# MVME-HBUT/Faster-OreFSDet

Measured on AMD Instinct MI355X. Metric: images/sec at 640x640 25-shot (eval FPS: model(inputs) + device sync per image, bs=1 per GPU), higher is better.
Workload: dtype f32

## Files before the change

### faster-orefsdet_amd/csrc/ore_common.h

```cpp
#pragma once
#include <hip/hip_runtime.h>
#include <stdint.h>
#include <stdio.h>
#include "ore_hip.h"

void ore_set_error(const char* fmt, ...);
void ore_note_wino(int v);
int ore_last_wino(void);
void ore_note_launch(int code, int split);
void ore_flop_count_add(double flops);

#define ORE_CHECK_ARG(cond, ...)              \
    do {                                      \
        if (!(cond)) {                        \
            ore_set_error(__VA_ARGS__);       \
            return ORE_EINVAL;                \
        }                                     \
    } while (0)

#define ORE_HIP(call)                                                                   \
    do {                                                                                \
        hipError_t e_ = (call);                                                         \
        if (e_ != hipSuccess) {                                                         \
            ore_set_error("%s:%d %s -> %s", __FILE__, __LINE__, #call, hipGetErrorString(e_)); \
            return ORE_EHIP;                                                            \
        }                                                                               \
    } while (0)

static inline int ore_launch_status(const char* what) {
    hipError_t e = hipGetLastError();
    if (e != hipSuccess) {
        ore_set_error("launch %s -> %s", what, hipGetErrorString(e));
        return ORE_EHIP;
    }
    return ORE_OK;
}

static inline int ceil_div(int a, int b) { return (a + b - 1) / b; }
static inline int round_up(int a, int b) { return ceil_div(a, b) * b; }

typedef float f32x4 __attribute__((ext_vector_type(4)));
typedef float f32x2 __attribute__((ext_vector_type(2)));
typedef __bf16 bf16x2_t __attribute__((ext_vector_type(2)));
typedef short s16x4 __attribute__((ext_vector_type(4)));
typedef unsigned u32x2 __attribute__((ext_vector_type(2)));

__device__ __forceinline__ s16x4 to_bf16x4(f32x4 v) {
    const bf16x2_t lo = __builtin_convertvector(f32x2{v.x, v.y}, bf16x2_t), hi = __builtin_convertvector(f32x2{v.z, v.w}, bf16x2_t);
    const u32x2 u = {__builtin_bit_cast(unsigned, lo), __builtin_bit_cast(unsigned, hi)};
    return __builtin_bit_cast(s16x4, u);
}

typedef __bf16 bf16x8_t __attribute__((ext_vector_type(8)));
__device__ __forceinline__ f32x4 from_bf16x4(s16x4 h) {
    const u32x2 u = __builtin_bit_cast(u32x2, h);
    return f32x4{__builtin_bit_cast(float, u.x << 16), __builtin_bit_cast(float, u.x & 0xffff0000u),
                 __builtin_bit_cast(float, u.y << 16), __builtin_bit_cast(float, u.y & 0xffff0000u)};
}
__device__ __forceinline__ float bf16_bits_to_f32(unsigned short h) { return __builtin_bit_cast(float, (unsigned)h << 16); }
struct ore_bf16_t { unsigned short v; };
__device__ __forceinline__ f32x4 ld4(const float* p) { return *reinterpret_cast<const f32x4*>(p); }
__device__ __forceinline__ f32x4 ld4(const ore_bf16_t* p) { return from_bf16x4(*reinterpret_cast<const s16x4*>(p)); }
__device__ __forceinline__ void st4(float* p, f32x4 v) { *reinterpret_cast<f32x4*>(p) = v; }
__device__ __forceinline__ void st4(ore_bf16_t* p, f32x4 v) { *reinterpret_cast<s16x4*>(p) = to_bf16x4(v); }
__device__ __forceinline__ float ld1(const float* p) { return *p; }
__device__ __forceinline__ float ld1(const ore_bf16_t* p) { return bf16_bits_to_f32(p->v); }

__device__ __forceinline__ __amdgpu_buffer_rsrc_t make_rsrc(const void* base, unsigned bytes) {
    return __builtin_amdgcn_make_buffer_rsrc(const_cast<void*>(base), 0, (int)bytes, 0x00020000);
}

__device__ __forceinline__ float ore_expf(float x) {
    if (x > 88.0f) x = 88.0f;
    if (x < -87.0f) x = -87.0f;
    const float n = rintf(x * 1.44269504088896341f);
    float r = fmaf(n, -0.693359375f, x);
    r = fmaf(n, 2.12194440e-4f, r);
    float p = 1.9875691500e-4f;
    p = fmaf(p, r, 1.3981999507e-3f);
    p = fmaf(p, r, 8.3334519073e-3f);
    p = fmaf(p, r, 4.1665795894e-2f);
    p = fmaf(p, r, 1.6666665459e-1f);
    p = fmaf(p, r, 5.0000001201e-1f);
    const float e = fmaf(p, r * r, r) + 1.0f;
    const int ni = (int)n;
    return e * __uint_as_float((unsigned)(ni + 127) << 23);
}

__device__ __forceinline__ float ore_sigmoid(float x) { return 1.0f / (1.0f + ore_expf(-x)); }

namespace oreroi {
int roi_predict_post(const float* h, int32_t C, int32_t h_parts, const float* h_bias, const float* cls_w, const float* cls_b,
                     const float* box_w, const float* box_b, const float* boxes, const int32_t* n_dev, int32_t n_host, int32_t cap,
                     const float* reg_weights4_host, float img_h, float img_w, float score_thresh, float nms_thresh,
                     int32_t topk, float* det_boxes, float* det_scores, int64_t* det_src, int32_t* det_count,
                     const float* post_dev, float* fin_boxes, float* fin_scores, int32_t* fin_count,
                     int32_t* host_count, void* workspace, size_t workspace_bytes, void* stream);
int roi_merge_classes(const float* det_boxes, const float* det_scores, const int32_t* det_count, int32_t K, int32_t cap,
                      const int64_t* class_ids, int32_t topk, const float* post_dev, float* fin_boxes, float* fin_scores,
                      int64_t* fin_classes, int32_t* fin_count, int32_t* host_count, void* stream);
struct PredictWs { size_t raw_boxes, c_boxes, raw_scores, c_scores, c_src, ok, keep, nms; };
inline PredictWs predict_ws_layout(int32_t cap) {
    const size_t c = (size_t)(cap > 0 ? cap : 1);
    PredictWs w{};
    size_t o = 256;
    w.raw_boxes = o; o += c * 16;
    w.c_boxes = o; o += c * 16;
    w.raw_scores = o; o += c * 4;
    w.c_scores = o; o += c * 4;
    w.c_src = o; o += c * 4;
    w.ok = o; o += c * 4;
    w.keep = o; o += c * 8;
    w.nms = (o + 255) & ~(size_t)255;
    return w;
}
}

namespace oremisc {
int correlation_classes(const float* q, int32_t q_ld, int32_t q_coff, int32_t n_levels, const int32_t* H, const int32_t* W, int32_t C,
                        int32_t K, const float* k11s, const float* k13s, const float* k31s, float* out, int32_t out_ld, void* stream);
int copy_cols(const float* src, int32_t src_ld, int32_t src_coff, int32_t rows, int32_t C, float* dst, int32_t dst_ld, void* stream);
}
```

### faster-orefsdet_amd/csrc/ore_detect.hip

```cpp
#include "ore_block.h"

#ifdef ORE_TRACE
__device__ unsigned long long* g_trace_det = nullptr;
#define DET_TR(i) do { if (g_trace_det && (i) < 512) g_trace_det[(i)] = __builtin_amdgcn_s_memtime(); } while (0)
__device__ int g_det_ablate = 0;
#define DET_ABL(bit) (g_det_ablate & (bit))
#else
#define DET_ABL(bit) 0
#define DET_TR(i) do { } while (0)
#endif

namespace {

struct DetP {
    int n_levels;
    const float* head[8]; int head_ld;
    int H[8], W[8], stride[8];
    float score_thresh; int pre_topk; float nms_thresh; int post_topk;
    int* lvl_cnt; float* lvl_boxes; float* lvl_scores; long long* lvl_loc;
    float* pre_boxes; float* pre_scores; long long* pre_loc; int* pre_level;
    float* s_boxes; float* s_scores; int* s_order;
    unsigned long long* mask; int mask_words;
    long long* keep_idx; int* counts; float* out_boxes; float* out_scores;
    int cap;
};

constexpr int SEL_T = 1024;
constexpr int NMS_MAX_WORDS = 256;

__device__ __forceinline__ int block_excl_scan(int v, int* lds_w, int* total) {
    const int lane = threadIdx.x & 63, wave = threadIdx.x >> 6;
    int inc = v;
#pragma unroll
    for (int d = 1; d < 64; d <<= 1) {
        const int t = __shfl_up(inc, d);
        if (lane >= d) inc += t;
    }
    __syncthreads();
    if (lane == 63) lds_w[wave] = inc;
    __syncthreads();
    int base = 0, tot = 0;
    for (int w = 0; w < SEL_T / 64; ++w) {
        const int s = lds_w[w];
        if (w < wave) base += s;
        tot += s;
    }
    *total = tot;
    return base + inc - v;
}

__device__ __forceinline__ void level_select_body(const DetP& p) {
    extern __shared__ __attribute__((aligned(16))) float sv[];
    __shared__ int hist[1024];
    __shared__ int wsum[SEL_T / 64];
    __shared__ int sh_i[4];
    const int l = blockIdx.x;
    const int HW = p.H[l] * p.W[l];
    const float* hd = p.head[l];
    const int tid = threadIdx.x;
    const bool tr = l == 0 && tid == 0;
    if (tr) DET_TR(0);

    int cnt = 0;
    for (int i = tid; i < HW; i += SEL_T) {
        const float s = ore_sigmoid(hd[(size_t)i * p.head_ld + 4]);
        sv[i] = s;
        cnt += s > p.score_thresh ? 1 : 0;
    }
    if (tr) DET_TR(1);
    int nc;
    block_excl_scan(cnt, wsum, &nc);
    if (tr) DET_TR(2);
    const int k = nc < p.pre_topk ? nc : p.pre_topk;

    unsigned T = 0;
    int quota = 0;
    bool take_all = true;
    if (nc > k) {
        take_all = false;
        unsigned prefix = 0, pmask = 0;
        int remaining = k;
        for (int pass = 0; pass < 3; ++pass) {
            const int shift = 20 - 10 * pass;
            for (int i = tid; i < 1024; i += SEL_T) hist[i] = 0;
            __syncthreads();
            for (int i = tid; i < HW; i += SEL_T) {
                const float s = sv[i];
                const unsigned key = __float_as_uint(s);
                if (s > p.score_thresh && (key & pmask) == prefix) atomicAdd(&hist[(key >> shift) & 1023], 1);
            }
            __syncthreads();
            if (tid < 64) {
                int h[16], t = 0;
#pragma unroll
                for (int j = 0; j < 16; ++j) { h[j] = hist[16 * tid + j]; t += h[j]; }
                int suf = t;
#pragma unroll
                for (int d = 1; d < 64; d <<= 1) {
                    const int o = __shfl_down(suf, d);
                    if (tid + d < 64) suf += o;
                }
                const int above = suf - t;
                if (suf >= remaining && above < remaining) {
                    int acc = above, dsel = 0, rem = remaining;
                    bool found = false;
#pragma unroll
                    for (int j = 15; j >= 0; --j) {
                        if (!found) {
                            if (acc + h[j] >= remaining) { dsel = j; rem = remaining - acc; found = true; }
                            else acc += h[j];
                        }
                    }
                    sh_i[0] = 16 * tid + dsel; sh_i[1] = rem;
                }
            }
            __syncthreads();
            prefix |= (unsigned)sh_i[0] << shift;
            pmask |= 1023u << shift;
            remaining = sh_i[1];
            if (tr) DET_TR(3 + pass);
        }
        T = prefix; quota = remaining;
    }

    const float st = (float)p.stride[l];
    const float half = (float)(p.stride[l] / 2);
    long long loc_base = 0;
    for (int j = 0; j < l; ++j) loc_base += (long long)p.H[j] * p.W[j];
    const int per = (HW + SEL_T - 1) / SEL_T;
    const int i_lo = min(tid * per, HW), i_hi = min(i_lo + per, HW);
    int my_gt = 0, my_tie = 0;
    for (int i = i_lo; i < i_hi; ++i) {
        const float s = sv[i];
        const bool cand = s > p.score_thresh;
        const unsigned key = __float_as_uint(s);
        my_gt += (cand && (take_all || key > T)) ? 1 : 0;
        my_tie += (cand && !take_all && key == T) ? 1 : 0;
    }
    if (tr) DET_TR(6);
    int tot;
    const int pre = block_excl_scan((my_gt << 16) | my_tie, wsum, &tot);
    if (tr) DET_TR(7);
    int tie_before = pre & 0xffff, gt_before = pre >> 16;
    for (int i = i_lo; i < i_hi; ++i) {
        const float s = sv[i];
        const bool cand = s > p.score_thresh;
        const unsigned key = __float_as_uint(s);
        const bool gt = cand && (take_all || key > T);
        const bool tie = cand && !take_all && key == T;
        if (gt || (tie && tie_before < quota)) {
            const int pos = gt_before + min(tie_before, quota);
            const float gx = (float)((i % p.W[l]) * p.stride[l]) + half;
            const float gy = (float)((i / p.W[l]) * p.stride[l]) + half;
            const f32x4 r = *reinterpret_cast<const f32x4*>(hd + (size_t)i * p.head_ld);
            const float x1 = gx - r.x * st, y1 = gy - r.y * st;
            float x2 = gx + r.z * st, y2 = gy + r.w * st;
            x2 = fmaxf(x2, x1 + 0.01f);
            y2 = fmaxf(y2, y1 + 0.01f);
            const size_t o = (size_t)l * p.pre_topk + pos;
            *reinterpret_cast<f32x4*>(p.lvl_boxes + o * 4) = f32x4{x1, y1, x2, y2};
            p.lvl_scores[o] = sqrtf(s);
            p.lvl_loc[o] = loc_base + i;
        }
        gt_before += gt ? 1 : 0;
        tie_before += tie ? 1 : 0;
    }
    const int out_base = (tot >> 16) + min(tot & 0xffff, quota);
    if (tid == 0) p.lvl_cnt[l] = out_base;
    if (tr) DET_TR(8);
}

__global__ __launch_bounds__(SEL_T) void k_level_select(DetP p) { level_select_body(p); }

constexpr int DET_BATCH = 16;
struct DetImg { const float* head[4]; char* ws; float* pre_boxes; float* pre_scores; long long* pre_loc; int* pre_level;
                long long* keep_idx; int* counts; float* out_boxes; float* out_scores; };
struct DetBatch {
    DetP common;
    size_t o_lvl_cnt, o_lvl_boxes, o_lvl_scores, o_lvl_loc, o_s_boxes, o_s_scores, o_s_order, o_mask;
    DetImg img[DET_BATCH];
};
__device__ __forceinline__ DetP det_of(const DetBatch& b, int i) {
    DetP p = b.common;
    const DetImg& m = b.img[i];
#pragma unroll
    for (int l = 0; l < 4; ++l) p.head[l] = m.head[l];
    p.lvl_cnt = (int*)(m.ws + b.o_lvl_cnt); p.lvl_boxes = (float*)(m.ws + b.o_lvl_boxes);
    p.lvl_scores = (float*)(m.ws + b.o_lvl_scores); p.lvl_loc = (long long*)(m.ws + b.o_lvl_loc);
    p.s_boxes = (float*)(m.ws + b.o_s_boxes); p.s_scores = (float*)(m.ws + b.o_s_scores); p.s_order = (int*)(m.ws + b.o_s_order);
    p.mask = (unsigned long long*)(m.ws + b.o_mask);
    p.pre_boxes = m.pre_boxes; p.pre_scores = m.pre_scores; p.pre_loc = m.pre_loc; p.pre_level = m.pre_level;
    p.keep_idx = m.keep_idx; p.counts = m.counts; p.out_boxes = m.out_boxes; p.out_scores = m.out_scores;
    return p;
}
__global__ __launch_bounds__(SEL_T) void k_level_select_b(DetBatch b) { const DetP p = det_of(b, blockIdx.y); level_select_body(p); }

__device__ __forceinline__ void rank_scatter_body(const DetP& p) {
    extern __shared__ float sc[];
    __shared__ int off[9];
    if (threadIdx.x == 0) {
        int a = 0;
        for (int l = 0; l < p.n_levels; ++l) { off[l] = a; a += p.lvl_cnt[l]; }
        off[p.n_levels] = a;
    }
    __syncthreads();
    const int n = off[p.n_levels];
    if (n == 0) {
        if (blockIdx.x == 0 && threadIdx.x == 0) p.counts[0] = 0;
        return;
    }
    if ((int)blockIdx.x * 16 >= n) return;
    for (int l = 0; l < p.n_levels; ++l)
        for (int i = threadIdx.x; i < off[l + 1] - off[l]; i += 256) sc[off[l] + i] = p.lvl_scores[(size_t)l * p.pre_topk + i];
    __syncthreads();
    const int e = blockIdx.x * 16 + (threadIdx.x >> 4), sub = threadIdx.x & 15;
    const bool valid = e < n;
    const float se = valid ? sc[e] : 0.f;
    int cntb = 0;
    if (valid)
        for (int f = sub; f < n; f += 16) {
            const float sf = sc[f];
            cntb += (sf > se || (sf == se && f < e)) ? 1 : 0;
        }
#pragma unroll
    for (int d = 8; d > 0; d >>= 1) cntb += __shfl_xor(cntb, d);
    if (valid && sub == 0) {
        int l = 0;
        while (e >= off[l + 1]) ++l;
        const size_t src = (size_t)l * p.pre_topk + (e - off[l]);
        const f32x4 b = *reinterpret_cast<const f32x4*>(p.lvl_boxes + src * 4);
        *reinterpret_cast<f32x4*>(p.pre_boxes + (size_t)e * 4) = b;
        p.pre_scores[e] = se;
        p.pre_loc[e] = p.lvl_loc[src];
        p.pre_level[e] = l;
        *reinterpret_cast<f32x4*>(p.s_boxes + (size_t)cntb * 4) = b;
        p.s_scores[cntb] = se;
        p.s_order[cntb] = e;
        if (e == 0) p.counts[0] = n;
    }
}

__global__ __launch_bounds__(256) void k_rank_scatter(DetP p) { rank_scatter_body(p); }
__global__ __launch_bounds__(256) void k_rank_scatter_b(DetBatch b) { const DetP p = det_of(b, blockIdx.y); rank_scatter_body(p); }

__device__ __forceinline__ void nms_mask_body(const float* __restrict__ boxes, const int* __restrict__ n_ptr,
                                              float thr, unsigned long long* __restrict__ mask, int words) {
    const int n = *n_ptr;
    const int bi = blockIdx.y, bj = blockIdx.x;
// ... 460 lines not shown

#ifdef ORE_TRACE
extern "C" int ore_debug_set_det_ablate(int flags) {
    ORE_HIP(hipMemcpyToSymbol(HIP_SYMBOL(g_det_ablate), &flags, sizeof(flags)));
    return ORE_OK;
}
extern "C" int ore_debug_set_trace_det(unsigned long long* buf) {
    ORE_HIP(hipMemcpyToSymbol(HIP_SYMBOL(g_trace_det), &buf, sizeof(buf)));
    return ORE_OK;
}
#endif

extern "C" size_t ore_detect_workspace_bytes(int32_t n_levels, int32_t pre_topk) {
    if (n_levels <= 0 || pre_topk <= 0) return 0;
    return det_layout(n_levels, pre_topk).total;
}

namespace {
static int detect_fill(const ore_detect_desc* d, DetP& p, DetLayout& lay, int& cap, size_t& sv_bytes) {
    ORE_CHECK_ARG(d && d->n_levels > 0 && d->n_levels <= 8 && d->pre_topk > 0, "ore_detect_fwd: bad args");
    ORE_CHECK_ARG(d->head_ld >= 8 && d->head_ld % 4 == 0, "ore_detect_fwd: head_ld=%d (need >= 8, %%4)", d->head_ld);
    ORE_CHECK_ARG(d->pre_boxes && d->pre_scores && d->pre_loc && d->pre_level && d->keep_idx && d->counts && d->out_boxes &&
                      d->out_scores && d->workspace, "ore_detect_fwd: null pointer");
    lay = det_layout(d->n_levels, d->pre_topk);
    if (d->workspace_bytes < lay.total) {
        ore_set_error("ore_detect_fwd: workspace %zu < %zu", d->workspace_bytes, lay.total);
        return ORE_ENOMEM;
    }
    cap = d->n_levels * d->pre_topk;
    ORE_CHECK_ARG((size_t)cap * 4 <= 150 * 1024 && lay.words <= NMS_MAX_WORDS, "ore_detect_fwd: cap %d too large", cap);
    ORE_CHECK_ARG(d->nms_thresh > 0.0f, "ore_detect_fwd: nms_thresh <= 0 (NMS disabled) is not supported");
    char* ws = (char*)d->workspace;
    p = DetP{};
    p.n_levels = d->n_levels; p.head_ld = d->head_ld;
    for (int l = 0; l < d->n_levels; ++l) {
        ORE_CHECK_ARG(d->head[l] && d->H[l] > 0 && d->W[l] > 0 && d->stride[l] > 0, "ore_detect_fwd: level %d", l);
        p.head[l] = d->head[l]; p.H[l] = d->H[l]; p.W[l] = d->W[l]; p.stride[l] = d->stride[l];
    }
    p.score_thresh = d->score_thresh; p.pre_topk = d->pre_topk; p.nms_thresh = d->nms_thresh; p.post_topk = d->post_topk;
    p.lvl_cnt = (int*)(ws + lay.lvl_cnt); p.lvl_boxes = (float*)(ws + lay.lvl_boxes);
    p.lvl_scores = (float*)(ws + lay.lvl_scores); p.lvl_loc = (long long*)(ws + lay.lvl_loc);
    p.pre_boxes = d->pre_boxes; p.pre_scores = d->pre_scores; p.pre_loc = (long long*)d->pre_loc; p.pre_level = d->pre_level;
    p.s_boxes = (float*)(ws + lay.s_boxes); p.s_scores = (float*)(ws + lay.s_scores); p.s_order = (int*)(ws + lay.s_order);
    p.mask = (unsigned long long*)(ws + lay.mask); p.mask_words = lay.words;
    p.keep_idx = (long long*)d->keep_idx; p.counts = d->counts; p.out_boxes = d->out_boxes; p.out_scores = d->out_scores;
    p.cap = cap;
    int hw_max = 0;
    for (int l = 0; l < d->n_levels; ++l) hw_max = max(hw_max, d->H[l] * d->W[l]);
    sv_bytes = (size_t)hw_max * 4;
    ORE_CHECK_ARG(sv_bytes <= 120 * 1024, "ore_detect_fwd: a level with %d locations exceeds the 30720-location LDS cache", hw_max);
    return ORE_OK;
}

static int detect_prepare(const ore_detect_desc* d, hipStream_t st, ScanArgs& sa, DetLayout& lay, int& cap) {
    DetP p{};
    size_t sv_bytes = 0;
    int rc = detect_fill(d, p, lay, cap, sv_bytes);
    if (rc) return rc;
    if (sv_bytes > 48 * 1024)
        ORE_HIP(hipFuncSetAttribute((const void*)k_level_select, hipFuncAttributeMaxDynamicSharedMemorySize, (int)sv_bytes));
    hipLaunchKernelGGL(k_level_select, dim3(d->n_levels), dim3(SEL_T), sv_bytes, st, p);
    if ((rc = ore_launch_status("k_level_select"))) return rc;
    const size_t sc_bytes = (size_t)cap * 4;
    if (sc_bytes > 64 * 1024)
        ORE_HIP(hipFuncSetAttribute((const void*)k_rank_scatter, hipFuncAttributeMaxDynamicSharedMemorySize, (int)sc_bytes));
    hipLaunchKernelGGL(k_rank_scatter, dim3(ceil_div(cap, 16)), dim3(256), sc_bytes, st, p);
    if ((rc = ore_launch_status("k_rank_scatter"))) return rc;
    if ((rc = launch_nms_mask(lay.words, cap, st, p.s_boxes, p.counts, d->nms_thresh, p.mask))) return rc;
    sa = ScanArgs{p.s_boxes, p.s_scores, p.s_order, p.counts, p.mask, p.keep_idx, p.out_boxes, p.out_scores, p.counts + 1};
    return ORE_OK;
}

static int detect_prepare_batch(const ore_detect_desc* d, int nb, hipStream_t st, ScanBatch& sb, DetLayout& lay, int& cap, bool& done) {
    done = false;
    if (nb < 2 || nb > DET_BATCH || d->n_levels > 4) return ORE_OK;
    DetBatch db{};
    size_t sv_bytes = 0;
    for (int i = 0; i < nb; ++i) {
        DetP p{};
        DetLayout li{};
        int ci = 0;
        size_t svi = 0;
        const int rc = detect_fill(d + i, p, li, ci, svi);
        if (rc) return rc;
        if (i == 0) { db.common = p; lay = li; cap = ci; sv_bytes = svi; if (nms_use_col(cap)) return ORE_OK; }
        const DetP& c = db.common;
        bool same = p.n_levels == c.n_levels && p.head_ld == c.head_ld && p.score_thresh == c.score_thresh && p.pre_topk == c.pre_topk;
        for (int l = 0; l < p.n_levels; ++l) same = same && p.H[l] == c.H[l] && p.W[l] == c.W[l] && p.stride[l] == c.stride[l];
        if (!same) return ORE_OK;
        DetImg& m = db.img[i];
        for (int l = 0; l < p.n_levels; ++l) m.head[l] = p.head[l];
        m.ws = (char*)d[i].workspace;
        m.pre_boxes = p.pre_boxes; m.pre_scores = p.pre_scores; m.pre_loc = p.pre_loc; m.pre_level = p.pre_level;
        m.keep_idx = p.keep_idx; m.counts = p.counts; m.out_boxes = p.out_boxes; m.out_scores = p.out_scores;
        sb.a[i] = ScanArgs{p.s_boxes, p.s_scores, p.s_order, p.counts, p.mask, p.keep_idx, p.out_boxes, p.out_scores, p.counts + 1};
    }
    db.o_lvl_cnt = lay.lvl_cnt; db.o_lvl_boxes = lay.lvl_boxes; db.o_lvl_scores = lay.lvl_scores; db.o_lvl_loc = lay.lvl_loc;
    db.o_s_boxes = lay.s_boxes; db.o_s_scores = lay.s_scores; db.o_s_order = lay.s_order; db.o_mask = lay.mask;
    int rc;
    if (sv_bytes > 48 * 1024)
        ORE_HIP(hipFuncSetAttribute((const void*)k_level_select_b, hipFuncAttributeMaxDynamicSharedMemorySize, (int)sv_bytes));
    hipLaunchKernelGGL(k_level_select_b, dim3(db.common.n_levels, nb), dim3(SEL_T), sv_bytes, st, db);
    if ((rc = ore_launch_status("k_level_select_b"))) return rc;
    const size_t sc_bytes = (size_t)cap * 4;
    if (sc_bytes > 64 * 1024)
        ORE_HIP(hipFuncSetAttribute((const void*)k_rank_scatter_b, hipFuncAttributeMaxDynamicSharedMemorySize, (int)sc_bytes));
    hipLaunchKernelGGL(k_rank_scatter_b, dim3(ceil_div(cap, 16), nb), dim3(256), sc_bytes, st, db);
    if ((rc = ore_launch_status("k_rank_scatter_b"))) return rc;
    hipLaunchKernelGGL(k_nms_mask_b, dim3(lay.words, lay.words, nb), dim3(256), 0, st, db, d->nms_thresh, lay.words);
    if ((rc = ore_launch_status("k_nms_mask_b"))) return rc;
    done = true;
    return ORE_OK;
}

}

extern "C" int ore_detect_fwd(const ore_detect_desc* d, void* stream) {
    ScanArgs sa{};
    DetLayout lay{};
    int cap = 0;
    hipStream_t st = (hipStream_t)stream;
    const int rc = detect_prepare(d, st, sa, lay, cap);
    if (rc) return rc;
    return launch_nms_scan(lay.words, st, sa.s_boxes, sa.s_scores, sa.s_order, sa.n_ptr, sa.mask, d->nms_thresh, d->post_topk, sa.keep_idx,
                           sa.out_boxes, sa.out_scores, sa.n_keep_out, nms_use_col(cap) ? nms_col_ld(cap) : 0);
}

extern "C" int ore_detect_batch_fwd(const ore_detect_desc* d, int32_t n_images, void* stream) {
    ORE_CHECK_ARG(d && n_images > 0, "ore_detect_batch_fwd: bad args");
    hipStream_t st = (hipStream_t)stream;
    for (int i0 = 0; i0 < n_images; i0 += SCAN_BATCH) {
        const int nb = min(SCAN_BATCH, n_images - i0);
        ScanBatch sb{};
        DetLayout lay{};
        int cap = 0;
        for (int i = 0; i < nb; ++i) {
            const ore_detect_desc* di = d + i0 + i;
            ORE_CHECK_ARG(di->n_levels == d->n_levels && di->pre_topk == d->pre_topk && di->nms_thresh == d->nms_thresh &&
                              di->post_topk == d->post_topk, "ore_detect_batch_fwd: image %d differs in levels / thresholds", i0 + i);
        }
        bool batched = false;
        { const int rc = detect_prepare_batch(d + i0, nb, st, sb, lay, cap, batched); if (rc) return rc; }
        for (int i = 0; i < nb && !batched; ++i) {
            const int rc = detect_prepare(d + i0 + i, st, sb.a[i], lay, cap);
            if (rc) return rc;
        }
        if (nms_use_col(cap) || nb == 1) {
            for (int i = 0; i < nb; ++i) {
                const ScanArgs& a = sb.a[i];
                const int rc = launch_nms_scan(lay.words, st, a.s_boxes, a.s_scores, a.s_order, a.n_ptr, a.mask, d->nms_thresh, d->post_topk,
                                               a.keep_idx, a.out_boxes, a.out_scores, a.n_keep_out, nms_use_col(cap) ? nms_col_ld(cap) : 0);
                if (rc) return rc;
            }
            continue;
        }
        sb.words = lay.words; sb.thr = d->nms_thresh; sb.post_topk = d->post_topk;
        const size_t dl = (size_t)lay.words * 64 * 8;
        const void* f = lay.words <= 64 ? (const void*)k_nms_scan_multi<1> : (lay.words <= 128 ? (const void*)k_nms_scan_multi<2> : (const void*)k_nms_scan_multi<4>);
        if (dl > 48 * 1024) ORE_HIP(hipFuncSetAttribute(f, hipFuncAttributeMaxDynamicSharedMemorySize, (int)dl));
        if (lay.words <= 64) hipLaunchKernelGGL(k_nms_scan_multi<1>, dim3(nb), dim3(256), dl, st, sb);
        else if (lay.words <= 128) hipLaunchKernelGGL(k_nms_scan_multi<2>, dim3(nb), dim3(256), dl, st, sb);
        else hipLaunchKernelGGL(k_nms_scan_multi<4>, dim3(nb), dim3(256), dl, st, sb);
        const int rc = ore_launch_status("k_nms_scan_multi");
        if (rc) return rc;
    }
    return ORE_OK;
}

namespace {
__global__ __launch_bounds__(256) void k_nms_prep(const float* __restrict__ boxes, const float* __restrict__ scores, int n_host,
                                                  const int* __restrict__ n_dev, float* s_boxes, float* s_scores, int* s_order,
                                                  int* n_out) {
    extern __shared__ float sc[];
    const int n = n_dev ? min(*n_dev, n_host) : n_host;
    for (int i = threadIdx.x; i < n; i += 256) sc[i] = scores[i];
    __syncthreads();
    const int e = blockIdx.x * 16 + (threadIdx.x >> 4), sub = threadIdx.x & 15;
    const bool valid = e < n;
// ... 79 lines not shown
```

### faster-orefsdet_amd/csrc/ore_engine.hip

```cpp
#include <map>
#include <string>
#include <vector>
#include <math.h>
#include <string.h>
#include "ore_common.h"
#include "ore_conv_internal.h"
#include <algorithm>


namespace {

struct HostTensor { std::vector<float> v; std::vector<int64_t> shape; };

struct Conv {
    float* w = nullptr; float* scale = nullptr; float* shift = nullptr;
    uint16_t* wh = nullptr;
    float* wino = nullptr;
    int Cin = 0, Cout = 0, k = 1, stride = 1, pad = 0, relu_cout = 0;
};

struct DwUnit { float* w_dw = nullptr; float* w_pw = nullptr; float* scale = nullptr; float* shift = nullptr; int C = 0, stride = 1; };

struct Buf { float* p = nullptr; int ld = 0; size_t rows = 0; };

struct Geo { int B, H, W, Hp, Wp; int h[6], w[6]; };

}

struct PrecisionScope {
    int saved;
    explicit PrecisionScope(int mode) : saved(ore_conv_get_precision()) { ore_conv_set_precision(mode); }
    ~PrecisionScope() { ore_conv_set_precision(saved); }
};

struct ore_engine {
    ore_model_cfg cfg{};
    int device = 0;
    int conv_precision = ORE_CONV_FP32;
    bool finalized = false;
    std::map<std::string, HostTensor> host;
    std::vector<void*> allocs;
    float* stem1_w = nullptr; float* stem1_scale = nullptr; float* stem1_shift = nullptr;
    Conv stem2, stem3;
    struct Block { Conv layer[8]; Conv concat; float* fc_w = nullptr; float* fc_b = nullptr; int cat_ch = 0; };
    struct Stage { Conv layer[8]; Conv concat; float* fc_w = nullptr; float* fc_b = nullptr; int in_ch, conv_ch, out_ch, cat_ch;
                   DwUnit dw[8]; Conv reduction; bool has_reduction = false; std::vector<Block> more; } stage[4];
    int blocks[4] = {1, 1, 1, 1};
    Buf icat[4][2], ycat[4];
    float* gate_blk = nullptr;
    bool depthwise = false;
    DwUnit dstem2, dstem3;
    Buf red[4];
    float* dw_scratch = nullptr; size_t dw_scratch_floats = 0;
    Conv lateral[3], output[3], conv3, tower, pred;
    float* out_wino3 = nullptr; float* out_shift3 = nullptr; size_t out_wino_stride = 0;
    uint16_t* out_wh3 = nullptr; size_t out_wh_stride = 0;
    float* gn_gamma = nullptr; float* gn_beta = nullptr;
    float* k11 = nullptr, *k13 = nullptr, *k31 = nullptr;
    HostTensor support[3];
    bool support_set[3] = {false, false, false};
    void* img_in = nullptr; size_t img_bytes = 0;
    Buf s1, s2, cat[4], sout[4], lat_all;
    Buf pcat, pos, tow, head;
    bool head_pred_valu = true;
    Buf tn;
    bool sb() const { return conv_precision == ORE_CONV_BF16S; }
    float* at(float* base, size_t elems) const { return sb() ? reinterpret_cast<float*>(reinterpret_cast<uint16_t*>(base) + elems) : base + elems; }
    float* gate[4] = {};
    float* lat_scaled[3] = {};
    float* gn_mul = nullptr, *gn_add = nullptr;
    float* ws = nullptr; size_t ws_floats = 0;
    float* ese_ws = nullptr;
    float* gn_ws = nullptr;
    float* colsum = nullptr; size_t colsum_floats = 0;
    float* pre_boxes = nullptr; float* pre_scores = nullptr; int64_t* pre_loc = nullptr; int32_t* pre_level = nullptr;
    int64_t* keep_idx = nullptr; int32_t* counts = nullptr; float* out_boxes = nullptr; float* out_scores = nullptr;
    void* det_ws = nullptr; size_t det_ws_bytes = 0;
    bool roi_set = false;
    int roi_cap = ORE_DET_RECORD_ROWS, roi_fc = 0, roi_pooled = 8, roi_topk = 100;
    float roi_score_thresh = 0.f, roi_nms_thresh = 0.9f, roi_reg_w[4] = {10.f, 10.f, 5.f, 5.f};
    float* roi_W = nullptr; float* roi_b = nullptr; float* roi_cls_w = nullptr; float* roi_cls_b = nullptr;
    float* roi_box_w = nullptr; float* roi_box_b = nullptr;
    float* roi_feat = nullptr; float* roi_h = nullptr;
    float* roi_hp = nullptr; int roi_ksplit = 1;
    float* det_boxes = nullptr; float* det_scores = nullptr; int64_t* det_src = nullptr; int32_t* det_count = nullptr;
    void* roi_ws = nullptr; size_t roi_ws_bytes = 0;
    int roi_stages = 1;
    float* casc_W[ORE_MAX_CASCADE] = {}; float* casc_b[ORE_MAX_CASCADE] = {}; float* casc_cls_w[ORE_MAX_CASCADE] = {};
    float* casc_cls_b[ORE_MAX_CASCADE] = {}; float* casc_box_w[ORE_MAX_CASCADE] = {}; float* casc_box_b[ORE_MAX_CASCADE] = {};
    float casc_reg_w[ORE_MAX_CASCADE][4] = {};
    float* casc_boxes[2] = {}; float* casc_sum = nullptr; uint8_t* casc_dead = nullptr;
    float* post = nullptr; float post_host[4] = {1.f, 1.f, 0.f, 0.f};
    char* fin_pack = nullptr; int32_t* fin_count = nullptr;
    float* fin_boxes_of(size_t b) const { return (float*)(fin_pack + b * (size_t)roi_cap * 28); }
    float* fin_scores_of(size_t b) const { return fin_boxes_of(b) + (size_t)roi_cap * 4; }
    int32_t* pin_count = nullptr; int32_t* pin_count_dev = nullptr; float* pin_post = nullptr;
    int n_classes = 0, n_slots = 0;
    int64_t* class_ids = nullptr;
    float* k11s = nullptr, *k13s = nullptr, *k31s = nullptr;
    bool slot_support_set[ORE_MAX_CLASSES][3] = {};
    float* roi_W_slot[ORE_MAX_CLASSES] = {}; float* roi_b_slot[ORE_MAX_CLASSES] = {};
    float* casc_W_slot[ORE_MAX_CLASSES][ORE_MAX_CASCADE] = {}; float* casc_b_slot[ORE_MAX_CLASSES][ORE_MAX_CASCADE] = {};
    char* det_ws_slots = nullptr;
    hipStream_t cap_stream = nullptr;
    struct GraphKey { int u8, H, W, B, K; hipGraphExec_t exec; };
    std::vector<GraphKey> graphs;
    Geo last{};
    long long pass_serial = 0;
    double last_flops = 0.0;
    bool profiling = false;
    std::vector<hipEvent_t> ev_pool;
    size_t ev_used = 0;
    struct EvSpan { size_t a, b; double flops; double flops_exec; };
    double last_profile_exec_flops = 0.0;
    std::vector<EvSpan> spans;
    hipEvent_t next_event() {
        if (ev_used == ev_pool.size()) { hipEvent_t e; if (hipEventCreate(&e) != hipSuccess) return nullptr; ev_pool.push_back(e); }
        return ev_pool[ev_used++];
    }

    template <typename T> int dalloc(T** p, size_t n) {
        void* q = nullptr;
        ORE_HIP(hipMalloc(&q, (n ? n : 1) * sizeof(T)));
        allocs.push_back(q);
        *p = (T*)q;
        return ORE_OK;
    }
    int upload(float** dst, const std::vector<float>& v) {
        int rc = dalloc(dst, v.size());
        if (rc) return rc;
// ... 292 lines not shown
                                                   reinterpret_cast<const uint16_t*>(e->sout[s].p), e->sout[s].ld, 0, g.h[k], g.w[k],
                                                   reinterpret_cast<uint16_t*>(nx.p), nx.ld, 0, st)
                      : ore_ese_gate_pool_fwd(e->colsum, cs_rows, g.h[k] * g.w[k], S.out_ch, S.fc_w, S.fc_b, e->gate[s], lw, lrows,
                                              s >= 1 ? e->lat_scaled[s - 1] : nullptr, e->sout[s].p, e->sout[s].ld, 0, g.h[k], g.w[k], nx.p,
                                              nx.ld, 0, st);
            pooled_next = true;
        } else if (cs_rows > 0 && s >= 1 && e->lat_scaled[s - 1]) {
            lat_scaled_ok[s - 1] = true;
            r.rc = sb ? ore_ese_gate_scaled_weight_bf16_fwd(e->colsum, cs_rows, g.h[k] * g.w[k], S.out_ch, S.fc_w, S.fc_b, e->gate[s], e->ese_ws,
                                                            e->lateral[s - 1].w, round_up(e->lateral[s - 1].Cout, 16),
                                                            reinterpret_cast<uint16_t*>(e->lat_scaled[s - 1]), st)
                      : ore_ese_gate_scaled_weight_fwd(e->colsum, cs_rows, g.h[k] * g.w[k], S.out_ch, S.fc_w, S.fc_b, e->gate[s], e->ese_ws,
                                                       e->lateral[s - 1].w, round_up(e->lateral[s - 1].Cout, 16), e->lat_scaled[s - 1], st);
        } else if (cs_rows > 0)
            r.rc = ore_ese_gate_from_colsum_fwd(e->colsum, cs_rows, 1, g.h[k] * g.w[k], S.out_ch, S.fc_w, S.fc_b, e->gate[s], e->ese_ws, st);
        else if (sb) { ore_set_error("bf16-storage engine: the eSE pool must come fused from the concat conv (one image per pass)"); r.rc = ORE_EINVAL; }
        else
            r.rc = ore_ese_gate_fwd(e->sout[s].p, e->sout[s].ld, 0, g.B, g.h[k] * g.w[k], S.out_ch, S.fc_w, S.fc_b, e->gate[s],
                                    e->ese_ws, st);
    }
    const int F = c.fpn_ch;
    float* lat[3];
    for (int l = 0; l < 3; ++l) lat[l] = e->at(e->lat_all.p, (size_t)lvl_row0(g, l) * F);
    const bool grouped = e->out_wino3 != nullptr || e->out_wh3 != nullptr;
    for (int l = 2; l >= 0 && !r.rc; --l) {
        const int k = l + 3, s = l + 1;
        const float* add = l < 2 ? lat[l + 1] : nullptr;
        if (lat_scaled_ok[l]) {
            Conv lc = e->lateral[l];
            lc.w = e->lat_scaled[l];
            lc.wh = reinterpret_cast<uint16_t*>(e->lat_scaled[l]);
            r.conv(lc, e->sout[s].p, e->sout[s].ld, 0, g.B, g.h[k], g.w[k], lat[l], F, 0, nullptr, nullptr, 0, add, F, 0);
        } else if (sb) {
            ore_set_error("bf16-storage engine: the lateral needs the gate-scaled weights (one image per pass)"); r.rc = ORE_EINVAL;
        } else {
            r.conv(e->lateral[l], e->sout[s].p, e->sout[s].ld, 0, g.B, g.h[k], g.w[k], lat[l], F, 0,
                   e->blocks[s] > 1 ? nullptr : e->gate[s], nullptr, 0, add, F, 0);
        }
        if (!grouped)
            r.conv(e->output[l], lat[l], F, 0, g.B, g.h[k], g.w[k], e->at(e->pcat.p, (size_t)lvl_row0(g, l) * 2 * F), 2 * F, F);
    }
    if (grouped && !r.rc) {
        const int H[3] = {g.h[3], g.h[4], g.h[5]}, W[3] = {g.w[3], g.w[4], g.w[5]};
        Conv oc = e->output[0];
        oc.wino = e->out_wino3; oc.shift = e->out_shift3;
        if (sb) oc.wh = e->out_wh3;
        r.conv_levels(oc, e->lat_all.p, F, 0, g.B, H, W, e->pcat.p, 2 * F, F, F, nullptr, nullptr, 0, false, sb ? 0 : e->out_wino_stride,
                      sb ? e->out_wh_stride : 0);
    }
    *flops = r.flops;
    return r.rc;
}

int run_heads(ore_engine* e, const Geo& g, hipStream_t st, double* flops, bool correlate = true) {
    const ore_model_cfg& c = e->cfg;
    const int F = c.fpn_ch;
    Run r{e, st};
    r.prof = e->profiling;
    const int H[3] = {g.h[3], g.h[4], g.h[5]}, W[3] = {g.w[3], g.w[4], g.w[5]};
    const int HW[3] = {H[0] * W[0], H[1] * W[1], H[2] * W[2]};
    const bool sb = e->sb();
    const double rows = (double)g.B * (HW[0] + HW[1] + HW[2]);
    if (correlate) {
        for (int l = 0; l < 3; ++l)
            if (!e->support_set[l]) { ore_set_error("support prototype for level %d not set", l + 3); return ORE_EINVAL; }
        r.rc = sb ? ore_correlation_levels_bf16_fwd(reinterpret_cast<const uint16_t*>(e->pcat.p), 2 * F, F, g.B, 3, H, W, F, e->k11, e->k13, e->k31,
                                                    reinterpret_cast<uint16_t*>(e->pcat.p), 2 * F, 0, st)
                  : ore_correlation_levels_fwd(e->pcat.p, 2 * F, F, g.B, 3, H, W, F, e->k11, e->k13, e->k31, e->pcat.p, 2 * F, 0, st);
        if (r.rc) return r.rc;
        r.flops += 2.0 * 8.0 * rows * F;
    }
    r.conv_levels(e->conv3, e->pcat.p, 2 * F, 0, g.B, H, W, e->pos.p, F, 0);
    r.conv_levels(e->tower, e->pos.p, F, 0, g.B, H, W, e->tow.p, F, 0);
    if (r.rc) return r.rc;
    if (F == 128 && e->head_pred_valu) {
        r.rc = sb ? ore_head_pred_gn_bf16_fwd(reinterpret_cast<const uint16_t*>(e->tow.p), F, g.B, 3, H, W, 32, 1e-5f, e->gn_gamma, e->gn_beta,
                                              e->pred.w, e->pred.scale, e->pred.shift, 16, e->head.p, 8, e->gn_ws, st)
                  : ore_head_pred_gn_fwd(e->tow.p, F, g.B, 3, H, W, 32, 1e-5f, e->gn_gamma, e->gn_beta, e->pred.w, e->pred.scale,
                                         e->pred.shift, 16, e->head.p, 8, e->gn_ws, st);
        r.flops += 2.0 * rows * 5.0 * F * 9.0;
        *flops = r.flops;
        return r.rc;
    }
    r.rc = sb ? ore_groupnorm_affine_levels_bf16_fwd(reinterpret_cast<const uint16_t*>(e->tow.p), F, 0, g.B, 3, HW, F, 32, 1e-5f, e->gn_gamma,
                                                     e->gn_beta, e->gn_mul, e->gn_add, e->gn_ws, st)
              : ore_groupnorm_affine_levels_fwd(e->tow.p, F, 0, g.B, 3, HW, F, 32, 1e-5f, e->gn_gamma, e->gn_beta, e->gn_mul, e->gn_add,
                                                e->gn_ws, st);
    if (r.rc) return r.rc;
    if (sb) {
        if (!r.rc) r.rc = ore_groupnorm_apply_levels_bf16_fwd(reinterpret_cast<const uint16_t*>(e->tow.p), F, 0, g.B, 3, HW, F, e->gn_mul, e->gn_add, 1,
                                                              reinterpret_cast<uint16_t*>(e->tn.p), st);
        if (r.rc) return r.rc;
        r.conv_levels(e->pred, e->tn.p, F, 0, g.B, H, W, e->head.p, 8, 0, 16, nullptr, nullptr, 0, true);
        *flops = r.flops;
        return r.rc;
    }
    r.conv_levels(e->pred, e->tow.p, F, 0, g.B, H, W, e->head.p, 8, 0, 16, e->gn_mul, e->gn_add, 1);
    *flops = r.flops;
    return r.rc;
}

void detect_desc(ore_engine* e, const Geo& g, int b, ore_detect_desc& d) {
    const ore_model_cfg& c = e->cfg;
    const size_t cap = (size_t)3 * c.pre_topk;
    d.n_levels = 3; d.head_ld = 8;
    for (int l = 0; l < 3; ++l) {
        d.head[l] = e->head.p + ((size_t)lvl_row0(g, l) + (size_t)b * g.h[l + 3] * g.w[l + 3]) * 8;
        d.H[l] = g.h[l + 3]; d.W[l] = g.w[l + 3]; d.stride[l] = c.strides[l];
    }
    d.score_thresh = c.score_thresh; d.pre_topk = c.pre_topk; d.nms_thresh = c.nms_thresh; d.post_topk = c.post_topk;
    d.pre_boxes = e->pre_boxes + b * cap * 4; d.pre_scores = e->pre_scores + b * cap; d.pre_loc = e->pre_loc + b * cap;
    d.pre_level = e->pre_level + b * cap; d.keep_idx = e->keep_idx + b * cap; d.counts = e->counts + b * 4;
    d.out_boxes = e->out_boxes + b * cap * 4; d.out_scores = e->out_scores + b * cap;
    d.workspace = e->det_ws; d.workspace_bytes = e->det_ws_bytes;
}

int run_detect(ore_engine* e, const Geo& g, hipStream_t st, int b = 0) {
    ore_detect_desc d{};
    detect_desc(e, g, b, d);
    return ore_detect_fwd(&d, st);
}

int run_detect_classes(ore_engine* e, const Geo& g, hipStream_t st, int K) {
    ore_detect_desc d[ORE_MAX_CLASSES];
    for (int k = 0; k < K; ++k) {
        d[k] = ore_detect_desc{};
        detect_desc(e, g, k, d[k]);
        if (k > 0) d[k].workspace = e->det_ws_slots + (size_t)(k - 1) * e->det_ws_bytes;
    }
    return ore_detect_batch_fwd(d, K, st);
}

static int run_roi_rows(ore_engine* e, const Geo& g, hipStream_t st, double* flops, int b, float* roi_W, float* roi_b, const float* out_boxes,
                        const int32_t* counts);

int run_roi(ore_engine* e, const Geo& g, hipStream_t st, double* flops, int b = 0, bool class_slot = false) {
    const ore_model_cfg& c = e->cfg;
    const size_t cap = (size_t)3 * c.pre_topk, rcap = (size_t)e->roi_cap;
    float* out_boxes = e->out_boxes + b * cap * 4;
    int32_t* counts = e->counts + b * 4;
    const int S = e->roi_ksplit, NS = e->roi_stages;
    const float* h = S > 1 ? e->roi_hp : e->roi_h;
    *flops = 0.0;
    const float* boxes_k = out_boxes;
    for (int k = 0; k < NS - 1; ++k) {
        float* W_k = k == 0 ? (class_slot ? e->roi_W_slot[b] : e->roi_W) : (class_slot ? e->casc_W_slot[b][k] : e->casc_W[k]);
        float* b_k = k == 0 ? (class_slot ? e->roi_b_slot[b] : e->roi_b) : (class_slot ? e->casc_b_slot[b][k] : e->casc_b[k]);
        double fl = 0.0;
        int rc = run_roi_rows(e, g, st, &fl, b, W_k, b_k, boxes_k, counts);
        if (rc) return rc;
        *flops += fl;
        float* next = e->casc_boxes[k & 1];
        rc = ore_roi_cascade_refine_fwd(h, e->roi_fc, S > 1 ? S : 0, S > 1 ? b_k : nullptr, k == 0 ? e->roi_cls_w : e->casc_cls_w[k],
                                        k == 0 ? e->roi_cls_b : e->casc_cls_b[k], k == 0 ? e->roi_box_w : e->casc_box_w[k],
                                        k == 0 ? e->roi_box_b : e->casc_box_b[k], boxes_k, counts + 1, 0, e->roi_cap,
                                        k == 0 ? e->roi_reg_w : e->casc_reg_w[k], (float)g.H, (float)g.W, next, e->casc_sum, e->casc_dead,
                                        k > 0 ? 1 : 0, st);
        if (rc) return rc;
        boxes_k = next;
    }
    const int kl = NS - 1;
    float* roi_W = kl == 0 ? (class_slot ? e->roi_W_slot[b] : e->roi_W) : (class_slot ? e->casc_W_slot[b][kl] : e->casc_W[kl]);
    float* roi_b = kl == 0 ? (class_slot ? e->roi_b_slot[b] : e->roi_b) : (class_slot ? e->casc_b_slot[b][kl] : e->casc_b[kl]);
    double fl = 0.0;
    int rc = run_roi_rows(e, g, st, &fl, b, roi_W, roi_b, boxes_k, counts);
    if (rc) return rc;
    *flops += fl;
    if (kl == 0)
        return oreroi::roi_predict_post(h, e->roi_fc, S > 1 ? S : 0, S > 1 ? roi_b : nullptr, e->roi_cls_w, e->roi_cls_b,
                                        e->roi_box_w, e->roi_box_b, out_boxes, counts + 1, 0,
                                        e->roi_cap, e->roi_reg_w, (float)g.H, (float)g.W, e->roi_score_thresh, e->roi_nms_thresh, e->roi_topk,
                                        e->det_boxes + b * rcap * 4, e->det_scores + b * rcap, e->det_src + b * rcap, e->det_count + b * 4,
// ... 107 lines not shown
extern "C" int ore_engine_set_roi_cascade(ore_engine* e, int32_t n_stages, const float* const* W_host, const float* const* b_host,
                                          int32_t fc_dim, int32_t pooled, const float* const* cls_w_host, const float* const* cls_b_host,
                                          const float* const* box_w_host, const float* const* box_b_host, const float* reg_weights4_host,
                                          float score_thresh, float nms_thresh, int32_t topk) {
    ORE_CHECK_ARG(e && W_host && b_host && cls_w_host && cls_b_host && box_w_host && box_b_host && reg_weights4_host,
                  "ore_engine_set_roi_cascade: null pointer");
    ORE_CHECK_ARG(n_stages >= 1 && n_stages <= ORE_MAX_CASCADE, "ore_engine_set_roi_cascade: %d cascade stages: the engine runs 1 .. %d", n_stages,
                  ORE_MAX_CASCADE);
    for (int k = 0; k < n_stages; ++k)
        ORE_CHECK_ARG(W_host[k] && b_host[k] && cls_w_host[k] && cls_b_host[k] && box_w_host[k] && box_b_host[k],
                      "ore_engine_set_roi_cascade: stage %d of %d: null pointer", k, n_stages);
    int rc = ore_engine_set_roi_head(e, W_host[0], b_host[0], fc_dim, pooled, cls_w_host[0], cls_b_host[0], box_w_host[0], box_b_host[0],
                                     reg_weights4_host, score_thresh, nms_thresh, topk);
    if (rc || n_stages == 1) return rc;
    const size_t K = (size_t)pooled * pooled * e->cfg.fpn_ch, cap = (size_t)e->roi_cap;
    auto up = [&](float** dst, const float* src, size_t n) -> int {
        if (!*dst && (rc = e->dalloc(dst, n))) return rc;
        ORE_HIP(hipMemcpy(*dst, src, n * sizeof(float), hipMemcpyHostToDevice));
        return ORE_OK;
    };
    for (int k = 1; k < n_stages; ++k) {
        if ((rc = up(&e->casc_W[k], W_host[k], (size_t)fc_dim * K)) || (rc = up(&e->casc_b[k], b_host[k], fc_dim)) ||
            (rc = up(&e->casc_cls_w[k], cls_w_host[k], 2 * (size_t)fc_dim)) || (rc = up(&e->casc_cls_b[k], cls_b_host[k], 2)) ||
            (rc = up(&e->casc_box_w[k], box_w_host[k], 4 * (size_t)fc_dim)) || (rc = up(&e->casc_box_b[k], box_b_host[k], 4)))
            return rc;
        for (int i = 0; i < 4; ++i) e->casc_reg_w[k][i] = reg_weights4_host[4 * k + i];
    }
    if (!e->casc_sum) {
        if ((rc = e->dalloc(&e->casc_boxes[0], cap * 4)) || (rc = e->dalloc(&e->casc_boxes[1], cap * 4)) || (rc = e->dalloc(&e->casc_sum, cap)) ||
            (rc = e->dalloc(&e->casc_dead, cap)))
            return rc;
        ORE_HIP(hipMemset(e->casc_boxes[0], 0, cap * 16));
        ORE_HIP(hipMemset(e->casc_boxes[1], 0, cap * 16));
        ORE_HIP(hipMemset(e->casc_sum, 0, cap * 4));
        ORE_HIP(hipMemset(e->casc_dead, 0, cap));
    }
    e->roi_stages = n_stages;
    ORE_HIP(hipDeviceSynchronize());
    return ORE_OK;
}

extern "C" int ore_engine_create(const ore_model_cfg* cfg, int32_t device, ore_engine** out) {
    ORE_CHECK_ARG(cfg && out, "ore_engine_create: null");
    ORE_CHECK_ARG(cfg->layers_per_block >= 1 && cfg->layers_per_block <= 8, "layers_per_block");
    ORE_CHECK_ARG(cfg->fpn_ch % 16 == 0 && cfg->max_batch >= 1 && cfg->max_h >= 32 && cfg->max_w >= 32, "bad cfg");
    for (int i = 0; i < 3; ++i) ORE_CHECK_ARG(cfg->stem_ch[i] % 16 == 0, "stem channels must be multiples of 16");
    for (int i = 0; i < 4; ++i)
        ORE_CHECK_ARG(cfg->stage_conv_ch[i] % 16 == 0 && cfg->stage_out_ch[i] % 16 == 0, "stage channels must be multiples of 16");
    ORE_HIP(hipSetDevice(device));
    ore_engine* e = new ore_engine();
    e->cfg = *cfg; e->device = device;
    e->conv_precision = ore_conv_get_precision();
    { const char* hm = getenv("ORE_HEAD_MFMA"); e->head_pred_valu = !(hm && hm[0] == '1'); }
    *out = e;
    return ORE_OK;
}

extern "C" void ore_engine_destroy(ore_engine* e) {
    if (!e) return;
    hipSetDevice(e->device);
    for (auto& g : e->graphs) hipGraphExecDestroy(g.exec);
    if (e->cap_stream) hipStreamDestroy(e->cap_stream);
    for (auto ev : e->ev_pool) hipEventDestroy(ev);
    for (void* p : e->allocs) hipFree(p);
    if (e->pin_count) hipHostFree(e->pin_count);
    if (e->pin_post) hipHostFree(e->pin_post);
    delete e;
}

extern "C" int ore_engine_set_tensor(ore_engine* e, const char* name, const float* data, const int64_t* shape, int32_t ndim) {
    ORE_CHECK_ARG(e && name && data && ndim >= 0 && ndim <= 8, "ore_engine_set_tensor: bad args");
    ORE_CHECK_ARG(!e->finalized, "ore_engine_set_tensor: engine already finalized");
    HostTensor t;
    size_t n = 1;
    for (int i = 0; i < ndim; ++i) { t.shape.push_back(shape[i]); n *= (size_t)shape[i]; }
    t.v.assign(data, data + n);
    e->host[name] = std::move(t);
    return ORE_OK;
}

extern "C" int ore_engine_set_support(ore_engine* e, int32_t level, const float* proto, int32_t C, int32_t s) {
    ORE_CHECK_ARG(e && proto && level >= 3 && level <= 5 && C == e->cfg.fpn_ch && s >= 1, "ore_engine_set_support: bad args");
    const int l = level - 3;
    e->support[l].v.assign(proto, proto + (size_t)C * s * s);
    e->support[l].shape = {C, s, s};
    if (e->finalized) {
        ORE_HIP(hipSetDevice(e->device));
        float* tmp = nullptr;
        ORE_HIP(hipMalloc((void**)&tmp, (size_t)C * s * s * sizeof(float)));
        hipError_t err = hipMemcpy(tmp, proto, (size_t)C * s * s * sizeof(float), hipMemcpyHostToDevice);
        int rc = err == hipSuccess ? ore_support_kernels_fwd(tmp, C, s, e->k11 + (size_t)l * C, e->k13 + (size_t)l * C * 3,
                                                             e->k31 + (size_t)l * C * 3, nullptr) : ORE_EHIP;
        hipDeviceSynchronize();
        hipFree(tmp);
        if (rc) return rc;
    }
    e->support_set[l] = true;
    return ORE_OK;
}

extern "C" int ore_engine_set_depthwise(ore_engine* e, int32_t on) {
    ORE_CHECK_ARG(e && !e->finalized, "ore_engine_set_depthwise: call it before ore_engine_finalize");
    ORE_CHECK_ARG(!on || !e->sb(), "ore_engine_set_depthwise: a bf16-storage engine has no depthwise body (the depthwise units are fp32 only)");
    ORE_CHECK_ARG(!on || (e->blocks[0] == 1 && e->blocks[1] == 1 && e->blocks[2] == 1 && e->blocks[3] == 1),
                  "ore_engine_set_depthwise: this engine has identity blocks (ore_engine_set_blocks): there is no deep depthwise body");
    e->depthwise = on != 0;
// ... 123 lines not shown
        if ((rc = e->upload(&p.w, packed))) return rc;
        p.Cin = F; p.Cout = 5; p.k = 3; p.stride = 1; p.pad = 1; p.relu_cout = 4;
        if ((rc = make_bf16_w(e, &p, w5.data()))) return rc;
        std::vector<float> scale(3 * 16, 0.f), shift(3 * 16, 0.f);
        for (int l = 0; l < 3; ++l) {
            const HostTensor* sc;
            if ((rc = need(e, hp + "scales." + std::to_string(l) + ".scale", &sc, {1}))) return rc;
            const float s = sc->v[0];
            for (int j = 0; j < 4; ++j) { scale[l * 16 + j] = s; shift[l * 16 + j] = br->v[j] * s; }
            scale[l * 16 + 4] = 1.0f; shift[l * 16 + 4] = bh->v[0];
        }
        if ((rc = e->upload(&p.scale, scale)) || (rc = e->upload(&p.shift, shift))) return rc;
    }
    const Geo g = make_geo(c.max_batch, c.max_h, c.max_w);
    const size_t B = g.B;
    e->img_bytes = B * 3 * (size_t)c.max_h * c.max_w * sizeof(float);
    ORE_HIP(hipMalloc(&e->img_in, e->img_bytes));
    e->allocs.push_back(e->img_in);
    if ((rc = alloc_buf(e, &e->s1, B * g.h[1] * g.w[1], c.stem_ch[0]))) return rc;
    if ((rc = alloc_buf(e, &e->s2, B * g.h[1] * g.w[1], c.stem_ch[1]))) return rc;
    size_t cmax = 0, cs_need = 0;
    for (int s = 0; s < 4; ++s) {
        const int k = s + 2;
        const size_t M = B * g.h[k] * g.w[k];
        if ((rc = alloc_buf(e, &e->cat[s], M, e->stage[s].cat_ch))) return rc;
        if ((rc = alloc_buf(e, &e->sout[s], M, e->stage[s].out_ch))) return rc;
        if (e->stage[s].has_reduction && (rc = alloc_buf(e, &e->red[s], M, e->stage[s].conv_ch))) return rc;
        if (e->depthwise && ore_dwpw_prefers_composition((int64_t)M, e->stage[s].conv_ch, 1))
            e->dw_scratch_floats = std::max(e->dw_scratch_floats, M * (size_t)e->stage[s].conv_ch);
        if ((rc = e->dalloc(&e->gate[s], B * e->stage[s].out_ch))) return rc;
        if (e->blocks[s] > 1) {
            const int icw = e->stage[s].out_ch + c.layers_per_block * e->stage[s].conv_ch;
            if ((rc = alloc_buf(e, &e->ycat[s], M, e->stage[s].out_ch)) || (rc = alloc_buf(e, &e->icat[s][0], M, icw))) return rc;
            if (e->blocks[s] > 2 && (rc = alloc_buf(e, &e->icat[s][1], M, icw))) return rc;
            const std::vector<float> ones(B * e->stage[s].out_ch, 1.0f);
            ORE_HIP(hipMemcpy(e->gate[s], ones.data(), ones.size() * sizeof(float), hipMemcpyHostToDevice));
        } else if (s >= 1 && (rc = e->dalloc(&e->lat_scaled[s - 1], (size_t)round_up(e->cfg.fpn_ch, 16) * e->stage[s].out_ch))) return rc;
        if ((size_t)e->stage[s].out_ch > cmax) cmax = e->stage[s].out_ch;
        const size_t cs = (M / 16 + 1) * (size_t)e->stage[s].out_ch;
        if (cs > cs_need) cs_need = cs;
    }
    if (e->depthwise) {
        const size_t m1 = B * g.h[1] * g.w[1];
        if (ore_dwpw_prefers_composition((int64_t)m1, c.stem_ch[1], 1)) e->dw_scratch_floats = std::max(e->dw_scratch_floats, m1 * (size_t)c.stem_ch[1]);
        if (e->dw_scratch_floats && (rc = e->dalloc(&e->dw_scratch, e->dw_scratch_floats))) return rc;
    }
    size_t rows_all = 0;
    for (int l = 0; l < 3; ++l) rows_all += (size_t)B * g.h[l + 3] * g.w[l + 3];
    if ((rc = alloc_buf(e, &e->lat_all, rows_all, F))) return rc;
    if ((rc = alloc_buf(e, &e->pcat, rows_all, 2 * F)) || (rc = alloc_buf(e, &e->pos, rows_all, F)) ||
        (rc = alloc_buf(e, &e->tow, rows_all, F)) || (rc = alloc_buf(e, &e->head, rows_all, 8, false))) return rc;
    if (e->sb() && (rc = alloc_buf(e, &e->tn, rows_all, F))) return rc;
    ORE_HIP(hipMemset(e->head.p, 0, rows_all * 8 * sizeof(float)));
    if ((rc = e->dalloc(&e->gn_mul, 3 * B * F)) || (rc = e->dalloc(&e->gn_add, 3 * B * F))) return rc;
    if ((rc = e->dalloc(&e->k11, (size_t)3 * F)) || (rc = e->dalloc(&e->k13, (size_t)3 * F * 3)) || (rc = e->dalloc(&e->k31, (size_t)3 * F * 3))) return rc;
    e->ws_floats = ore_conv_workspace_floats();
    if ((rc = e->dalloc(&e->ws, e->ws_floats))) return rc;
    ORE_HIP(hipMemset(e->ws, 0, e->ws_floats * sizeof(float)));
    if ((rc = e->dalloc(&e->ese_ws, B * (ORE_ESE_PARTS + 1) * cmax))) return rc;
    if (std::any_of(e->blocks, e->blocks + 4, [](int n) { return n > 1; }) && (rc = e->dalloc(&e->gate_blk, B * cmax))) return rc;
    e->colsum_floats = cs_need;
    if ((rc = e->dalloc(&e->colsum, cs_need))) return rc;
    if ((rc = e->dalloc(&e->gn_ws, (rows_all / 64 + 3 * B + 8) * 64 * 2))) return rc;
    const size_t cap = (size_t)3 * c.pre_topk;
    const size_t MB = (size_t)c.max_batch;
    if ((rc = e->dalloc(&e->pre_boxes, MB * cap * 4)) || (rc = e->dalloc(&e->pre_scores, MB * cap)) || (rc = e->dalloc(&e->pre_loc, MB * cap)) ||
        (rc = e->dalloc(&e->pre_level, MB * cap)) || (rc = e->dalloc(&e->keep_idx, MB * cap)) || (rc = e->dalloc(&e->counts, MB * 4)) ||
        (rc = e->dalloc(&e->out_boxes, MB * cap * 4)) || (rc = e->dalloc(&e->out_scores, MB * cap))) return rc;
    ORE_HIP(hipMemset(e->counts, 0, MB * 4 * sizeof(int32_t)));
    e->det_ws_bytes = ore_detect_workspace_bytes(3, c.pre_topk);
    char* dws = nullptr;
    if ((rc = e->dalloc(&dws, e->det_ws_bytes))) return rc;
    e->det_ws = dws;
    ORE_HIP(hipStreamCreateWithFlags(&e->cap_stream, hipStreamNonBlocking));
    e->finalized = true;
    for (int l = 0; l < 3; ++l)
        if (!e->support[l].v.empty()) {
            e->support_set[l] = false;
            if ((rc = ore_engine_set_support(e, l + 3, e->support[l].v.data(), (int)e->support[l].shape[0], (int)e->support[l].shape[1]))) return rc;
        }
    e->host.clear();
    ORE_HIP(hipDeviceSynchronize());
    return ORE_OK;
}

static int check_geo(ore_engine* e, int B, int H, int W) {
    ORE_CHECK_ARG(e && e->finalized, "engine not finalized");
    ORE_CHECK_ARG(B >= 1 && B <= e->cfg.max_batch && H >= 1 && W >= 1 && round_up(H, 32) <= round_up(e->cfg.max_h, 32) &&
                      round_up(W, 32) <= round_up(e->cfg.max_w, 32) &&
                      (size_t)B * round_up(H, 32) * round_up(W, 32) <= (size_t)e->cfg.max_batch * round_up(e->cfg.max_h, 32) * round_up(e->cfg.max_w, 32),
                  "input %dx%dx%d exceeds the engine's max %dx%dx%d", B, H, W, e->cfg.max_batch, e->cfg.max_h, e->cfg.max_w);
    return ORE_OK;
}

template <typename Body>
static int replay_or_capture(ore_engine* e, int is_u8, int H, int W, int B, int K, hipStream_t st, Body& body) {
    for (auto& k : e->graphs)
        if (k.u8 == is_u8 && k.H == H && k.W == W && k.B == B && k.K == K) {
            ORE_HIP(hipGraphLaunch(k.exec, st));
            return ORE_OK;
        }
    hipGraph_t graph = nullptr;
    const bool was_prof = e->profiling;
    e->profiling = false;
    ORE_HIP(hipStreamBeginCapture(e->cap_stream, hipStreamCaptureModeThreadLocal));
    int rc = body(e->cap_stream, &e->last_flops);
// ... 51 lines not shown

extern "C" int ore_engine_detect_begin(ore_engine* e, const void* img, int32_t is_u8, int32_t H, int32_t W, int32_t out_h, int32_t out_w,
                                       void* out_record, void* stream) {
    return detect_begin(e, img, is_u8, H, W, out_h, out_w, out_record, stream, false);
}

extern "C" int ore_engine_detect_end(ore_engine* e, void* stream, int32_t* n_det) {
    ORE_CHECK_ARG(e && e->roi_set && n_det, "ore_engine_detect_end: null");
    hipStream_t st = (hipStream_t)stream;
    volatile unsigned long long* rec_word = reinterpret_cast<volatile unsigned long long*>(e->pin_count) + 1;
    volatile int32_t* cnt_word = e->pin_count;
    ORE_CHECK_ARG(*rec_word != 0ull, "ore_engine_detect_end: no ore_engine_detect_begin is pending on this engine");
    int32_t n = -1;
    for (int spin = 0; spin < (1 << 22); ++spin) {
        n = *cnt_word;
        if (n >= 0) break;
        __builtin_ia32_pause();
    }
    if (n < 0) {
        const hipError_t se = hipStreamSynchronize(st);
        if (se != hipSuccess) { *rec_word = 0ull; ore_set_error("ore_engine_detect_end: %s", hipGetErrorString(se)); return ORE_EHIP; }
        n = *cnt_word;
        if (n < 0) { *rec_word = 0ull; ore_set_error("ore_engine_detect_end: the pass finished without writing the detection count"); return ORE_EHIP; }
    }
    __atomic_thread_fence(__ATOMIC_ACQUIRE);
    *rec_word = 0ull;
    *n_det = n;
    return ORE_OK;
}

extern "C" int ore_engine_detect_fwd(ore_engine* e, const void* img, int32_t is_u8, int32_t H, int32_t W, int32_t out_h, int32_t out_w,
                                     void* out_record, void* stream, int32_t* n_det) {
    ORE_CHECK_ARG(n_det, "ore_engine_detect_fwd: null count");
    const int rc = ore_engine_detect_begin(e, img, is_u8, H, W, out_h, out_w, out_record, stream);
    return rc ? rc : ore_engine_detect_end(e, stream, n_det);
}

extern "C" int ore_engine_eval_batch_fwd(ore_engine* e, const void* img, int32_t is_u8, int32_t B, int32_t H, int32_t W,
                                         int32_t use_graph, void* stream) {
    int rc = check_geo(e, B, H, W);
    if (rc) return rc;
    ORE_CHECK_ARG(img, "null image");
    hipStream_t st = (hipStream_t)stream;
    const Geo g = make_geo(B, H, W);
    e->last = g; ++e->pass_serial;
    PrecisionScope ps(e->sb() ? ORE_CONV_FP32 : e->conv_precision);
    const size_t bytes = (size_t)B * 3 * H * W * (is_u8 ? 1 : 4);
    ORE_CHECK_ARG(bytes <= e->img_bytes, "image batch exceeds the engine's input buffer");
    if (img != e->img_in) ORE_HIP(hipMemcpyAsync(e->img_in, img, bytes, hipMemcpyDefault, st));
    auto body = [&](hipStream_t s, double* fl) -> int {
        double f1 = 0, f2 = 0;
        int r = run_backbone(e, e->img_in, is_u8, g, s, &f1);
        double f3 = 0;
        if (!r) r = run_heads(e, g, s, &f2);
        for (int b = 0; b < B && !r; ++b) {
            double fb = 0;
            r = run_detect(e, g, s, b);
            if (!r && e->roi_set) r = run_roi(e, g, s, &fb, b);
            f3 += fb;
        }
        *fl = f1 + f2 + f3;
        return r;
    };
    if (!use_graph) return body(st, &e->last_flops);
    return replay_or_capture(e, is_u8, H, W, B, 0, st, body);
}

static int eval_classes(ore_engine* e, const void* img, int32_t is_u8, int32_t H, int32_t W, int32_t use_graph, hipStream_t st) {
    ORE_CHECK_ARG(e && e->finalized, "engine not finalized");
    const int K = e->n_classes;
    ORE_CHECK_ARG(K >= 1, "N-way pass: no class set (ore_engine_set_classes with n >= 1 first)");
    for (int k = 0; k < K; ++k) {
        for (int l = 0; l < 3; ++l)
            ORE_CHECK_ARG(e->slot_support_set[k][l], "N-way pass: class slot %d has no support prototype for level %d (ore_engine_set_support_slot)", k, l + 3);
        ORE_CHECK_ARG(!e->roi_set || e->roi_W_slot[k], "N-way pass: class slot %d has no second-stage support (ore_engine_set_roi_support_slot)", k);
        for (int sk = 1; sk < e->roi_stages && e->roi_set; ++sk)
            ORE_CHECK_ARG(e->casc_W_slot[k][sk], "N-way pass: class slot %d has no second-stage support for stage %d of the %d cascade stages "
                          "(ore_engine_set_roi_support_slot_stage)", k, sk, e->roi_stages);
    }
    int rc = check_geo(e, K, H, W);
    if (rc) return rc;
    ORE_CHECK_ARG(img, "null image");
    const Geo g1 = make_geo(1, H, W), gK = make_geo(K, H, W);
    e->last = gK; ++e->pass_serial;
    PrecisionScope ps(e->conv_precision);
    const size_t bytes = (size_t)3 * H * W * (is_u8 ? 1 : 4);
    ORE_CHECK_ARG(bytes <= e->img_bytes, "image exceeds the engine's input buffer");
    if (img != e->img_in) ORE_HIP(hipMemcpyAsync(e->img_in, img, bytes, hipMemcpyDefault, st));
    const int F = e->cfg.fpn_ch;
    auto body = [&](hipStream_t s, double* fl) -> int {
        double f1 = 0, f2 = 0, f3 = 0;
        int r = run_backbone(e, e->img_in, is_u8, g1, s, &f1);
        const int rows1 = lvl_row0(g1, 3);
        const int Hl[3] = {g1.h[3], g1.h[4], g1.h[5]}, Wl[3] = {g1.w[3], g1.w[4], g1.w[5]};
        if (!r) r = oremisc::copy_cols(e->pcat.p, 2 * F, F, rows1, F, e->tow.p, F, s);
        if (!r) r = oremisc::correlation_classes(e->tow.p, F, 0, 3, Hl, Wl, F, K, e->k11s, e->k13s, e->k31s, e->pcat.p, 2 * F, s);
        f2 += 2.0 * 8.0 * (double)K * rows1 * F;
        double fh = 0;
        if (!r) r = run_heads(e, gK, s, &fh, false);
        f2 += fh;
        if (!r) r = run_detect_classes(e, gK, s, K);
        for (int k = 0; k < K && !r && e->roi_set; ++k) {
            double fb = 0;
            r = run_roi(e, gK, s, &fb, k, true);
            f3 += fb;
        }
        if (!r && e->roi_set)
// ... 134 lines not shown
extern "C" int ore_event_pair_overhead_us(void* stream, int32_t reps, double* median_us) {
    ORE_CHECK_ARG(median_us && reps >= 1 && reps <= 4096, "ore_event_pair_overhead_us: bad args");
    hipStream_t st = (hipStream_t)stream;
    std::vector<hipEvent_t> ev(2 * (size_t)reps);
    for (auto& e : ev) ORE_HIP(hipEventCreate(&e));
    double T[2] = {0.0, 0.0};
    for (int nk = 1; nk <= 2; ++nk) {
        for (int i = 0; i < 8; ++i) hipLaunchKernelGGL(k_noop, dim3(256), dim3(256), 0, st);
        for (int i = 0; i < reps; ++i) {
            ORE_HIP(hipEventRecord(ev[2 * i], st));
            for (int k = 0; k < nk; ++k) hipLaunchKernelGGL(k_noop, dim3(256), dim3(256), 0, st);
            ORE_HIP(hipEventRecord(ev[2 * i + 1], st));
        }
        ORE_HIP(hipStreamSynchronize(st));
        std::vector<float> t((size_t)reps);
        for (int i = 0; i < reps; ++i) ORE_HIP(hipEventElapsedTime(&t[i], ev[2 * i], ev[2 * i + 1]));
        std::sort(t.begin(), t.end());
        T[nk - 1] = 1e3 * (double)t[t.size() / 2];
    }
    for (auto& e : ev) (void)hipEventDestroy(e);
    const double o = 2.0 * T[0] - T[1];
    *median_us = o > 0.0 ? o : 0.0;
    return ORE_OK;
}

extern "C" int ore_engine_buffer(ore_engine* e, const char* name, void** ptr, int64_t dims[4]) {
    ORE_CHECK_ARG(e && e->finalized && name && ptr && dims, "ore_engine_buffer: bad args");
    const Geo& g = e->last;
    const std::string n(name);
    const int F = e->cfg.fpn_ch;
    auto set = [&](void* p, int64_t rows, int64_t ch, int64_t ld, int64_t coff) {
        *ptr = p; dims[0] = rows; dims[1] = ch; dims[2] = ld; dims[3] = coff; return ORE_OK;
    };
    const int64_t cap = (int64_t)3 * e->cfg.pre_topk;
    if (n == "stem1") return set(e->s1.p, (int64_t)g.B * g.h[1] * g.w[1], e->cfg.stem_ch[0], e->s1.ld, 0);
    if (n == "stem2") return set(e->s2.p, (int64_t)g.B * g.h[1] * g.w[1], e->cfg.stem_ch[1], e->s2.ld, 0);
    if (n == "stem3") return set(e->cat[0].p, (int64_t)g.B * g.h[2] * g.w[2], e->cfg.stem_ch[2], e->cat[0].ld, 0);
    for (int s = 0; s < 4; ++s) {
        const int64_t rows = (int64_t)g.B * g.h[s + 2] * g.w[s + 2];
        if (n == "stage" + std::to_string(s + 2)) return set(e->sout[s].p, rows, e->stage[s].out_ch, e->sout[s].ld, 0);
        if (n == "gate" + std::to_string(s + 2)) return set(e->gate[s], g.B, e->stage[s].out_ch, e->stage[s].out_ch, 0);
        if (n == "cat" + std::to_string(s + 2)) return set(e->cat[s].p, rows, e->stage[s].cat_ch, e->cat[s].ld, 0);
    }
    for (int l = 0; l < 3; ++l) {
        const std::string k = std::to_string(l + 3);
        const int64_t rows = (int64_t)g.B * g.h[l + 3] * g.w[l + 3];
        const size_t r0 = (size_t)lvl_row0(g, l);
        if (n == "p" + k) return set(e->at(e->pcat.p, r0 * 2 * F), rows, F, 2 * F, F);
        if (n == "attn" + k) return set(e->at(e->pcat.p, r0 * 2 * F), rows, F, 2 * F, 0);
        if (n == "lat" + k) return set(e->at(e->lat_all.p, r0 * F), rows, F, F, 0);
        if (n == "pos" + k) return set(e->at(e->pos.p, r0 * F), rows, F, F, 0);
        if (n == "tower" + k) return set(e->at(e->tow.p, r0 * F), rows, F, F, 0);
        if (n == "head" + k) return set(e->head.p + r0 * 8, rows, 5, 8, 0);
    }
    size_t ib = 0;
    std::string base = n;
    { const size_t h = n.find('#'); if (h != std::string::npos) { base = n.substr(0, h); ib = (size_t)std::atoi(n.c_str() + h + 1); } }
    if (ib >= (size_t)e->cfg.max_batch) { ore_set_error("ore_engine_buffer: image index in '%s' exceeds max_batch", name); return ORE_EINVAL; }
    const size_t ucap = (size_t)cap, rcap = (size_t)e->roi_cap;
    if (base == "pre_boxes") return set(e->pre_boxes + ib * ucap * 4, cap, 4, 4, 0);
    if (base == "pre_scores") return set(e->pre_scores + ib * ucap, cap, 1, 1, 0);
    if (base == "pre_loc") return set(e->pre_loc + ib * ucap, cap, 1, 1, 0);
    if (base == "pre_level") return set(e->pre_level + ib * ucap, cap, 1, 1, 0);
    if (base == "keep_idx") return set(e->keep_idx + ib * ucap, cap, 1, 1, 0);
    if (base == "counts") return set(e->counts + ib * 4, 4, 1, 1, 0);
    if (base == "out_boxes") return set(e->out_boxes + ib * ucap * 4, cap, 4, 4, 0);
    if (base == "out_scores") return set(e->out_scores + ib * ucap, cap, 1, 1, 0);
    if (e->roi_set) {
        if (base == "det_boxes") return set(e->det_boxes + ib * rcap * 4, e->roi_cap, 4, 4, 0);
        if (base == "det_scores") return set(e->det_scores + ib * rcap, e->roi_cap, 1, 1, 0);
        if (base == "det_src") return set(e->det_src + ib * rcap, e->roi_cap, 1, 1, 0);
        if (base == "det_count") return set(e->det_count + ib * 4, 4, 1, 1, 0);
        if (base == "final_boxes") return set(e->fin_boxes_of(ib), e->roi_cap, 4, 4, 0);
        if (base == "final_scores") return set(e->fin_scores_of(ib), e->roi_cap, 1, 1, 0);
        if (base == "final_count") return set(e->fin_count + ib * 4, 4, 1, 1, 0);
        if (base == "final_classes") return set(e->fin_pack + ib * rcap * 28 + rcap * 20, e->roi_cap, 1, 1, 0);
        if (n == "roi_h" && e->roi_ksplit <= 1) return set(e->roi_h, e->roi_cap, e->roi_fc, e->roi_fc, 0);
        const oreroi::PredictWs L = oreroi::predict_ws_layout(e->roi_cap);
        if (n == "roi_raw_boxes") return set((float*)((char*)e->roi_ws + L.raw_boxes), e->roi_cap, 4, 4, 0);
        if (n == "roi_raw_scores") return set((float*)((char*)e->roi_ws + L.raw_scores), e->roi_cap, 1, 1, 0);
        if (n == "roi_ok") return set((float*)((char*)e->roi_ws + L.ok), e->roi_cap, 1, 1, 0);
    }
    ore_set_error("ore_engine_buffer: unknown buffer '%s'", name);
    return ORE_ENOENT;
}

extern "C" int ore_engine_last_geometry(ore_engine* e, int32_t out[16]) {
    ORE_CHECK_ARG(e && e->finalized && out, "ore_engine_last_geometry: bad args");
    const Geo& g = e->last;
    out[0] = g.B; out[1] = g.H; out[2] = g.W;
    for (int l = 0; l < 3; ++l) { out[3 + 3 * l] = g.h[l + 3]; out[4 + 3 * l] = g.w[l + 3]; out[5 + 3 * l] = e->cfg.strides[l]; }
    out[12] = (int32_t)(e->pass_serial & 0x7fffffffLL); out[13] = (int32_t)(e->pass_serial >> 31);
    out[14] = out[15] = 0;
    return ORE_OK;
}

extern "C" int32_t ore_engine_buffer_is_bf16(ore_engine* e, const char* name) {
    if (!e || !name || !e->sb()) return 0;
    const std::string n(name);
    for (const char* pre : {"stem", "stage", "cat", "attn", "lat", "pos", "tower"})
        if (n.rfind(pre, 0) == 0) return 1;
    return n.size() == 2 && n[0] == 'p' ? 1 : 0;
}
```

### faster-orefsdet_amd/csrc/ore_misc.hip

```cpp
#include "ore_common.h"
#include "ore_ese.h"
#include <stdlib.h>
#include <algorithm>

namespace {

template <typename T, int NT, typename TO = float>
__global__ __launch_bounds__(256) void k_stem1(const T* __restrict__ img, int B, int H, int W, int Ho, int Wo,
                                               float m0, float m1, float m2, float s0, float s1, float s2,
                                               const float* __restrict__ w, const float* __restrict__ scale,
                                               const float* __restrict__ shift, int Cout, TO* __restrict__ out,
                                               int out_ld, int out_coff, int groups_per_wave) {
    constexpr int MAXNT = NT;
    const int lane = threadIdx.x & 63, wave = threadIdx.x >> 6;
    const int li = lane & 15, g = lane >> 4;
    int kdy[7], kdx[7], koff[7];
    bool kv[7];
    float kmean[7], kstd[7];
#pragma unroll
    for (int j = 0; j < 7; ++j) {
        const int k = 4 * j + g;
        kv[j] = k < 27;
        const int kk = kv[j] ? k : 0;
        const int kc = kk / 9;
// ... 375 lines not shown
struct GnSeg { int nlev, B; int HW[4]; int row0[4]; int chunk0[4]; int nchunk[4]; };

__device__ __forceinline__ void gn_locate_chunk(const GnSeg& g, int chunk, int& seg, int& HW, int& row0, int& local) {
    int l = 0;
#pragma unroll
    for (int j = 1; j < 4; ++j)
        if (j < g.nlev && chunk >= g.chunk0[j]) l = j;
    const int within = chunk - g.chunk0[l];
    const int b = within / g.nchunk[l];
    local = within - b * g.nchunk[l];
    HW = g.HW[l];
    row0 = g.row0[l] + b * HW;
    seg = l * g.B + b;
}

__global__ __launch_bounds__(256) void k_gn_chunk_stats(const float* __restrict__ x, int ld, int coff, GnSeg sg, int C, int G,
                                                        float* __restrict__ stats ) {
    __shared__ float red[256];
    __shared__ float gmean[64];
    int seg, HW, row0, chunk;
    gn_locate_chunk(sg, blockIdx.x, seg, HW, row0, chunk);
    const int cpg = C / G;
    const int rpar = 256 / C;
    const int c = threadIdx.x % C, rr = threadIdx.x / C;
    const int r0 = chunk * GN_ROWS, r1 = min(r0 + GN_ROWS, HW);
    const float* base = x + (size_t)row0 * ld + coff + c;
    float s = 0.f;
    for (int r = r0 + rr; r < r1; r += rpar) s += base[(size_t)r * ld];
    red[threadIdx.x] = s;
    __syncthreads();
    if (threadIdx.x < G) {
        float t = 0.f;
        for (int k = 0; k < rpar; ++k)
            for (int j = 0; j < cpg; ++j) t += red[k * C + threadIdx.x * cpg + j];
        gmean[threadIdx.x] = t / (float)((r1 - r0) * cpg);
    }
    __syncthreads();
    const float mu = gmean[c / cpg];
    float v = 0.f;
    for (int r = r0 + rr; r < r1; r += rpar) { const float d = base[(size_t)r * ld] - mu; v += d * d; }
    red[threadIdx.x] = v;
    __syncthreads();
    if (threadIdx.x < G) {
        float t = 0.f;
        for (int k = 0; k < rpar; ++k)
            for (int j = 0; j < cpg; ++j) t += red[k * C + threadIdx.x * cpg + j];
        float* o = stats + ((size_t)blockIdx.x * G + threadIdx.x) * 2;
        o[0] = gmean[threadIdx.x]; o[1] = t;
    }
}

template <int RPT, typename TS = float>
__global__ __launch_bounds__(256) void k_gn_chunk_stats4(const TS* __restrict__ x, int ld, int coff, GnSeg sg, int G,
                                                         float* __restrict__ stats ) {
    __shared__ float red[256];
    __shared__ float gmean[64];
    int seg, HW, row0, chunk;
    gn_locate_chunk(sg, blockIdx.x, seg, HW, row0, chunk);
    const int g = threadIdx.x % G, rr = threadIdx.x / G, rpar = 256 / G;
    const int r0 = chunk * GN_ROWS, r1 = min(r0 + GN_ROWS, HW);
    const TS* base = x + (size_t)row0 * ld + coff + g * 4;
    f32x4 v[RPT];
    float s = 0.f;
#pragma unroll
    for (int k = 0; k < RPT; ++k) {
        const int r = r0 + rr + k * rpar;
        v[k] = r < r1 ? ld4(base + (size_t)r * ld) : f32x4{0.f, 0.f, 0.f, 0.f};
        s += (v[k].x + v[k].y) + (v[k].z + v[k].w);
    }
    red[threadIdx.x] = s;
    __syncthreads();
    if (threadIdx.x < G) {
        float t = 0.f;
        for (int k = 0; k < rpar; ++k) t += red[k * G + threadIdx.x];
        gmean[threadIdx.x] = t / (float)((r1 - r0) * 4);
    }
    __syncthreads();
    const float mu = gmean[g];
    float q = 0.f;
#pragma unroll
    for (int k = 0; k < RPT; ++k) {
        if (r0 + rr + k * rpar < r1) {
            const float a = v[k].x - mu, b = v[k].y - mu, c = v[k].z - mu, d = v[k].w - mu;
            q += (a * a + b * b) + (c * c + d * d);
        }
    }
    red[threadIdx.x] = q;
    __syncthreads();
    if (threadIdx.x < G) {
        float t = 0.f;
        for (int k = 0; k < rpar; ++k) t += red[k * G + threadIdx.x];
        float* o = stats + ((size_t)blockIdx.x * G + threadIdx.x) * 2;
        o[0] = gmean[threadIdx.x]; o[1] = t;
    }
}

struct GnCombineSm { float sn[8][64], sm[8][64], sq[8][64], fmean[64], frstd[64]; };
__device__ __forceinline__ void gn_combine_block(GnCombineSm& S, const float* __restrict__ stats, const GnSeg& sg, int b, int C, int G, float eps,
                                                 const float* __restrict__ gamma, const float* __restrict__ beta, float* omul, float* oadd) {
    const int lvl = b / sg.B, img = b - lvl * sg.B;
    const int nchunks = sg.nchunk[lvl], HW = sg.HW[lvl];
    stats += (size_t)(sg.chunk0[lvl] + img * nchunks) * G * 2;
    const int cpg = C / G;
    const int gdiv = G > 32 ? 64 : 32, nsl = 256 / gdiv;
    const int g = threadIdx.x % gdiv, sl = threadIdx.x / gdiv;
    float n = 0.f, mean = 0.f, m2 = 0.f;
    if (g < G)
        for (int c0 = sl; c0 < nchunks; c0 += nsl * 8) {
            float2 rec[8];
// ... 6 lines not shown
            for (int k = 0; k < 8; ++k) {
                const int ch = c0 + nsl * k;
                if (ch < nchunks) {
                    const float nb = (float)((min((ch + 1) * GN_ROWS, HW) - ch * GN_ROWS) * cpg);
                    const float mb = rec[k].x, qb = rec[k].y;
                    const float nt = n + nb, d = mb - mean;
                    mean += d * (nb / nt);
                    m2 += qb + d * d * (n * nb / nt);
                    n = nt;
                }
            }
        }
    S.sn[sl][g] = n; S.sm[sl][g] = mean; S.sq[sl][g] = m2;
    __syncthreads();
    if (threadIdx.x < G) {
        float N = S.sn[0][g], M = S.sm[0][g], Q = S.sq[0][g];
        for (int k = 1; k < nsl; ++k) {
            const float nb = S.sn[k][g];
            if (nb > 0.f) {
                const float nt = N + nb, d = S.sm[k][g] - M;
                M += d * (nb / nt);
                Q += S.sq[k][g] + d * d * (N * nb / nt);
                N = nt;
            }
        }
        S.fmean[g] = M;
        S.frstd[g] = 1.0f / sqrtf(Q / N + eps);
    }
    __syncthreads();
    for (int c = threadIdx.x; c < C; c += 256) {
        const float m = S.frstd[c / cpg] * gamma[c];
        omul[c] = m;
        oadd[c] = beta[c] - S.fmean[c / cpg] * m;
    }
}

__global__ __launch_bounds__(256) void k_gn_combine(const float* __restrict__ stats, GnSeg sg, int C, int G, float eps,
                                                    const float* __restrict__ gamma, const float* __restrict__ beta,
                                                    float* __restrict__ mul, float* __restrict__ add) {
    __shared__ GnCombineSm S;
    const int b = blockIdx.x;
    gn_combine_block(S, stats, sg, b, C, G, eps, gamma, beta, mul + (size_t)b * C, add + (size_t)b * C);
}


struct HeadP {
    const void* tow; int ld;
    int B, nlev; int H[4], W[4], row0[4], tile0[5], tx[4], ty[4];
    const float* mul; const float* add;
    const float* w;
    const float* scale; const float* shift; int ep_stride;
    float* out; int out_ld;
    const float* stats; GnSeg sg; const float* gamma; const float* beta; float eps; int G;
};

template <typename TS>
__global__ __launch_bounds__(256) void k_head_pred(HeadP p) {
    constexpr int C = 128, Q = 32, NO = 5, TP = 8, HP = TP + 2;
    __shared__ __attribute__((aligned(16))) float sX[HP * HP * C];
    __shared__ __attribute__((aligned(16))) float sW[NO * 9 * C];
    const int tid = threadIdx.x;
    int lvl = 0;
#pragma unroll
    for (int l = 1; l < 4; ++l)
        if (l < p.nlev && (int)blockIdx.x >= p.tile0[l]) lvl = l;
    const int H = p.H[lvl], W = p.W[lvl];
    const int tl = blockIdx.x - p.tile0[lvl], per = p.tx[lvl] * p.ty[lvl];
    const int b = tl / per, tr = tl - b * per;
    const int y0 = (tr / p.tx[lvl]) * TP, x0 = (tr % p.tx[lvl]) * TP;
    const int base = p.row0[lvl] + b * H * W;
    const TS* tow = reinterpret_cast<const TS*>(p.tow);
    __shared__ __attribute__((aligned(16))) float s_mul[C], s_add[C];
    __shared__ GnCombineSm S;
    constexpr int NX = (HP * HP * Q + 255) / 256;
    constexpr int NWV = (NO * 9 * Q + 255) / 256;
    f32x4 xv[NX], wv[NWV];
#pragma unroll
    for (int k = 0; k < NWV; ++k) {
        const int i = tid + k * 256;
        wv[k] = i < NO * 9 * Q ? *reinterpret_cast<const f32x4*>(p.w + i * 4) : f32x4{0.f, 0.f, 0.f, 0.f};
    }
#pragma unroll
    for (int k = 0; k < NX; ++k) {
        const int i = tid + k * 256;
        const int px = i / Q, q = i - px * Q;
        const int gy = y0 - 1 + px / HP, gx = x0 - 1 + px % HP;
        const bool ok = i < HP * HP * Q && (unsigned)gy < (unsigned)H && (unsigned)gx < (unsigned)W;
        xv[k] = ok ? ld4(tow + (size_t)(base + gy * W + gx) * p.ld + q * 4) : f32x4{0.f, 0.f, 0.f, 0.f};
    }
    if (p.stats) gn_combine_block(S, p.stats, p.sg, lvl * p.B + b, C, p.G, p.eps, p.gamma, p.beta, s_mul, s_add);
    else if (tid < C) { s_mul[tid] = p.mul[(size_t)(lvl * p.B + b) * C + tid]; s_add[tid] = p.add[(size_t)(lvl * p.B + b) * C + tid]; }
    __syncthreads();
    const float* mul = s_mul;
    const float* add = s_add;
#pragma unroll
    for (int k = 0; k < NWV; ++k) {
        const int i = tid + k * 256;
        if (i < NO * 9 * Q) *reinterpret_cast<f32x4*>(sW + i * 4) = wv[k];
    }
#pragma unroll
    for (int k = 0; k < NX; ++k) {
        const int i = tid + k * 256;
        if (i < HP * HP * Q) {
            const int px = i / Q, q = i - px * Q;
            const int gy = y0 - 1 + px / HP, gx = x0 - 1 + px % HP;
            f32x4 v = {0.f, 0.f, 0.f, 0.f};
            if ((unsigned)gy < (unsigned)H && (unsigned)gx < (unsigned)W) {
                v = xv[k] * *reinterpret_cast<const f32x4*>(mul + q * 4) + *reinterpret_cast<const f32x4*>(add + q * 4);
                v.x = fmaxf(v.x, 0.f); v.y = fmaxf(v.y, 0.f); v.z = fmaxf(v.z, 0.f); v.w = fmaxf(v.w, 0.f);
            }
            *reinterpret_cast<f32x4*>(sX + i * 4) = v;
        }
    }
    __syncthreads();
    const int q = tid & 31, r = tid >> 5;
    float acc[TP][NO];
#pragma unroll
    for (int x = 0; x < TP; ++x)
#pragma unroll
        for (int o = 0; o < NO; ++o) acc[x][o] = 0.f;
#pragma unroll
    for (int dy = 0; dy < 3; ++dy) {
        f32x4 xr[HP];
#pragma unroll
        for (int x = 0; x < HP; ++x) xr[x] = *reinterpret_cast<const f32x4*>(sX + (((r + dy) * HP + x) * Q + q) * 4);
#pragma unroll
        for (int dx = 0; dx < 3; ++dx)
#pragma unroll
            for (int o = 0; o < NO; ++o) {
                const f32x4 w4 = *reinterpret_cast<const f32x4*>(sW + ((o * 9 + dy * 3 + dx) * Q + q) * 4);
#pragma unroll
                for (int x = 0; x < TP; ++x) {
                    const f32x4 v = xr[x + dx];
                    acc[x][o] = fmaf(v.x, w4.x, fmaf(v.y, w4.y, fmaf(v.z, w4.z, fmaf(v.w, w4.w, acc[x][o]))));
                }
            }
    }
    __syncthreads();
    float* part = sX;
#pragma unroll
    for (int x = 0; x < TP; ++x)
#pragma unroll
        for (int o = 0; o < NO; ++o) part[((r * TP + x) * NO + o) * Q + q] = acc[x][o];
    __syncthreads();
    for (int i = tid; i < TP * TP * NO; i += 256) {
        const int px = i / NO, o = i - px * NO;
        const float* pp = part + i * Q;
        float s0 = 0.f, s1 = 0.f, s2 = 0.f, s3 = 0.f;
#pragma unroll
        for (int k = 0; k < Q; k += 4) { s0 += pp[k]; s1 += pp[k + 1]; s2 += pp[k + 2]; s3 += pp[k + 3]; }
        float v = (s0 + s1) + (s2 + s3);
        const int gy = y0 + px / TP, gx = x0 + px % TP;
        if (gy < H && gx < W) {
            v = v * p.scale[lvl * p.ep_stride + o] + p.shift[lvl * p.ep_stride + o];
            if (o < 4) v = fmaxf(v, 0.f);
            p.out[(size_t)(base + gy * W + gx) * p.out_ld + o] = v;
        }
    }
}

}

struct HeadGn { const float* stats; GnSeg sg; const float* gamma; const float* beta; float eps; int G; };
static int head_pred_launch(const void* tower, int32_t ld, int32_t B, int32_t n_levels, const int32_t* H, const int32_t* W, const float* mul,
                            const float* add, const float* w_packed16, const float* scale, const float* shift, int32_t ep_stride,
                            float* out, int32_t out_ld, void* stream, int bf16, const HeadGn* gn = nullptr) {
    ORE_CHECK_ARG(tower && H && W && (gn || (mul && add)) && w_packed16 && scale && shift && out, "ore_head_pred_fwd: null pointer");
    ORE_CHECK_ARG(B > 0 && n_levels >= 1 && n_levels <= 4 && ld >= 128 && ld % 4 == 0 && out_ld >= 5, "ore_head_pred_fwd: bad args");
    HeadP p{};
    p.tow = tower; p.ld = ld; p.B = B; p.nlev = n_levels;
    int rows = 0, tiles = 0;
    for (int l = 0; l < n_levels; ++l) {
        ORE_CHECK_ARG(H[l] > 0 && W[l] > 0, "ore_head_pred_fwd: level %d geometry", l);
        p.H[l] = H[l]; p.W[l] = W[l]; p.row0[l] = rows; p.tile0[l] = tiles;
        p.tx[l] = ceil_div(W[l], 8); p.ty[l] = ceil_div(H[l], 8);
        rows += B * H[l] * W[l]; tiles += B * p.tx[l] * p.ty[l];
    }
    p.tile0[n_levels] = tiles;
    p.mul = mul; p.add = add; p.w = w_packed16; p.scale = scale; p.shift = shift; p.ep_stride = ep_stride; p.out = out; p.out_ld = out_ld;
    if (gn) { p.stats = gn->stats; p.sg = gn->sg; p.gamma = gn->gamma; p.beta = gn->beta; p.eps = gn->eps; p.G = gn->G; }
    if (bf16) hipLaunchKernelGGL(k_head_pred<ore_bf16_t>, dim3(tiles), dim3(256), 0, (hipStream_t)stream, p);
    else hipLaunchKernelGGL(k_head_pred<float>, dim3(tiles), dim3(256), 0, (hipStream_t)stream, p);
    return ore_launch_status("k_head_pred");
}

extern "C" int ore_head_pred_fwd(const float* tower, int32_t ld, int32_t B, int32_t n_levels, const int32_t* H, const int32_t* W,
                                 const float* gn_mul, const float* gn_add, const float* w_packed16, const float* scale, const float* shift,
                                 int32_t ep_stride, float* out, int32_t out_ld, void* stream) {
    return head_pred_launch(tower, ld, B, n_levels, H, W, gn_mul, gn_add, w_packed16, scale, shift, ep_stride, out, out_ld, stream, 0);
}

extern "C" int ore_head_pred_bf16_fwd(const uint16_t* tower, int32_t ld, int32_t B, int32_t n_levels, const int32_t* H, const int32_t* W,
                                      const float* gn_mul, const float* gn_add, const float* w_packed16, const float* scale,
                                      const float* shift, int32_t ep_stride, float* out, int32_t out_ld, void* stream) {
    return head_pred_launch(tower, ld, B, n_levels, H, W, gn_mul, gn_add, w_packed16, scale, shift, ep_stride, out, out_ld, stream, 1);
}

static int stem1_launch(const void* img, int32_t img_is_u8, int32_t B, int32_t H, int32_t W, int32_t Hp,
                             int32_t Wp, const float* mean3, const float* std3, const float* w_oihw,
                             const float* scale, const float* shift, int32_t Cout, void* out, int32_t out_ld,
                             int32_t out_coff, void* stream, int out_bf16) {
    ORE_CHECK_ARG(img && mean3 && std3 && w_oihw && scale && shift && out, "ore_stem1_fwd: null pointer");
    ORE_CHECK_ARG(B > 0 && H > 0 && W > 0 && Hp >= H && Wp >= W && Hp % 2 == 0 && Wp % 2 == 0, "ore_stem1_fwd: geometry");
    ORE_CHECK_ARG(Cout % 16 == 0 && Cout <= 128 && out_coff % 4 == 0 && out_ld % 4 == 0 && out_coff + Cout <= out_ld,
                  "ore_stem1_fwd: Cout=%d ld=%d coff=%d", Cout, out_ld, out_coff);
    const int Ho = Hp / 2, Wo = Wp / 2;
    const int M = B * Ho * Wo;
    ore_flop_count_add(2.0 * (double)M * Cout * 27.0);
    ORE_CHECK_ARG((long long)Ho * Wo < (1ll << 22) && (long long)B * Ho * Wo < (1ll << 31) && (long long)B * 3 * H * W < (1ll << 31),
                  "ore_stem1_fwd: %d images of %dx%d exceed the kernel's 32-bit indexing", B, H, W);
    hipStream_t st = (hipStream_t)stream;
    const int ngroups = ceil_div(M, 16);
    const int gpw = ngroups >= 2048 ? 2 : 1;
    const int blocks = ceil_div(ngroups, 4 * gpw);
#define ORE_STEM1(T, NT)                                                                                              \
    do { if (out_bf16) hipLaunchKernelGGL((k_stem1<T, NT, ore_bf16_t>), dim3(blocks), dim3(256), 0, st, (const T*)img, B, H, W, Ho, Wo, mean3[0], mean3[1], \
                       mean3[2], std3[0], std3[1], std3[2], w_oihw, scale, shift, Cout, (ore_bf16_t*)out, out_ld, out_coff, gpw); \
    else hipLaunchKernelGGL((k_stem1<T, NT, float>), dim3(blocks), dim3(256), 0, st, (const T*)img, B, H, W, Ho, Wo, mean3[0], mean3[1], \
                       mean3[2], std3[0], std3[1], std3[2], w_oihw, scale, shift, Cout, (float*)out, out_ld, out_coff, gpw); } while (0)
    switch ((Cout >> 4) * 2 + (img_is_u8 ? 1 : 0)) {
        case 2: ORE_STEM1(float, 1); break;     case 3: ORE_STEM1(uint8_t, 1); break;
        case 4: ORE_STEM1(float, 2); break;     case 5: ORE_STEM1(uint8_t, 2); break;
        case 8: ORE_STEM1(float, 4); break;     case 9: ORE_STEM1(uint8_t, 4); break;
        case 16: ORE_STEM1(float, 8); break;    case 17: ORE_STEM1(uint8_t, 8); break;
        default: ore_set_error("ore_stem1_fwd: Cout=%d not in {16,32,64,128}", Cout); return ORE_EINVAL;
    }
#undef ORE_STEM1
    return ore_launch_status("k_stem1");
}

extern "C" int ore_stem1_fwd(const void* img, int32_t img_is_u8, int32_t B, int32_t H, int32_t W, int32_t Hp,
                             int32_t Wp, const float* mean3, const float* std3, const float* w_oihw,
                             const float* scale, const float* shift, int32_t Cout, float* out, int32_t out_ld,
// ... 148 lines not shown
extern "C" int ore_correlation_fwd(const float* q, int32_t q_ld, int32_t q_coff, int32_t B, int32_t H, int32_t W,
                                   int32_t C, const float* k11, const float* k13, const float* k31, float* out,
                                   int32_t out_ld, int32_t out_coff, void* stream) {
    ORE_CHECK_ARG(q && k11 && k13 && k31 && out, "ore_correlation_fwd: null pointer");
    ORE_CHECK_ARG(C % 4 == 0 && q_ld % 4 == 0 && q_coff % 4 == 0 && out_ld % 4 == 0 && out_coff % 4 == 0,
                  "ore_correlation_fwd: alignment");
    CorrP p{};
    p.q = q; p.q_ld = q_ld; p.q_coff = q_coff; p.B = B; p.C4 = C / 4; p.nlev = 1; p.lv[0] = {0, H, W}; p.rows = B * H * W;
    p.k11 = k11; p.k13 = k13; p.k31 = k31; p.kstride = 0; p.out = out; p.out_ld = out_ld; p.out_coff = out_coff;
    hipLaunchKernelGGL(k_correlation<float>, dim3(ceil_div(p.rows * p.C4, 256)), dim3(256), 0, (hipStream_t)stream, p);
    return ore_launch_status("k_correlation");
}

extern "C" int ore_correlation_levels_fwd(const float* q, int32_t q_ld, int32_t q_coff, int32_t B, int32_t n_levels,
                                          const int32_t* H, const int32_t* W, int32_t C, const float* k11, const float* k13,
                                          const float* k31, float* out, int32_t out_ld, int32_t out_coff, void* stream) {
    ORE_CHECK_ARG(q && k11 && k13 && k31 && out && H && W && n_levels >= 1 && n_levels <= 4, "ore_correlation_levels_fwd: bad args");
    ORE_CHECK_ARG(C % 4 == 0 && q_ld % 4 == 0 && q_coff % 4 == 0 && out_ld % 4 == 0 && out_coff % 4 == 0,
                  "ore_correlation_levels_fwd: alignment");
    CorrP p{};
    p.q = q; p.q_ld = q_ld; p.q_coff = q_coff; p.B = B; p.C4 = C / 4; p.nlev = n_levels;
    int rows = 0;
    for (int l = 0; l < n_levels; ++l) { p.lv[l] = {rows, H[l], W[l]}; rows += B * H[l] * W[l]; }
    p.rows = rows;
    p.k11 = k11; p.k13 = k13; p.k31 = k31; p.kstride = C; p.out = out; p.out_ld = out_ld; p.out_coff = out_coff;
    hipLaunchKernelGGL(k_correlation<float>, dim3(ceil_div(p.rows * p.C4, 256)), dim3(256), 0, (hipStream_t)stream, p);
    return ore_launch_status("k_correlation");
}

extern "C" int ore_correlation_levels_bf16_fwd(const uint16_t* q, int32_t q_ld, int32_t q_coff, int32_t B, int32_t n_levels,
                                               const int32_t* H, const int32_t* W, int32_t C, const float* k11, const float* k13,
                                               const float* k31, uint16_t* out, int32_t out_ld, int32_t out_coff, void* stream) {
    ORE_CHECK_ARG(q && k11 && k13 && k31 && out && H && W && n_levels >= 1 && n_levels <= 4, "ore_correlation_levels_bf16_fwd: bad args");
    ORE_CHECK_ARG(C % 4 == 0 && q_ld % 4 == 0 && q_coff % 4 == 0 && out_ld % 4 == 0 && out_coff % 4 == 0,
                  "ore_correlation_levels_bf16_fwd: alignment");
    CorrP p{};
    p.q = q; p.q_ld = q_ld; p.q_coff = q_coff; p.B = B; p.C4 = C / 4; p.nlev = n_levels;
    int rows = 0;
    for (int l = 0; l < n_levels; ++l) { p.lv[l] = {rows, H[l], W[l]}; rows += B * H[l] * W[l]; }
    p.rows = rows;
    p.k11 = k11; p.k13 = k13; p.k31 = k31; p.kstride = C; p.out = out; p.out_ld = out_ld; p.out_coff = out_coff;
    hipLaunchKernelGGL(k_correlation<ore_bf16_t>, dim3(ceil_div(p.rows * p.C4, 256)), dim3(256), 0, (hipStream_t)stream, p);
    return ore_launch_status("k_correlation");
}

extern "C" int ore_support_kernels_fwd(const float* proto_chw, int32_t C, int32_t s, float* k11, float* k13,
                                       float* k31, void* stream) {
    ORE_CHECK_ARG(proto_chw && k11 && k13 && k31 && C > 0 && s >= 1, "ore_support_kernels_fwd: bad args");
    hipLaunchKernelGGL(k_support_kernels, dim3(C), dim3(64), 0, (hipStream_t)stream, proto_chw, s, k11, k13, k31);
    return ore_launch_status("k_support_kernels");
}

static int gn_stats_levels(const void* xv, int32_t ld, int32_t coff, int32_t B, int32_t n_levels, const int32_t* HW, int32_t C, int32_t groups,
                           float* workspace, hipStream_t st, int x_bf16, GnSeg* out_sg) {
    const float* x = (const float*)xv;
    ORE_CHECK_ARG(x && HW && workspace && n_levels >= 1 && n_levels <= 4 && groups > 0 && groups <= 64 && C % groups == 0 && C <= 256 &&
                      256 % C == 0, "ore_groupnorm_affine_levels_fwd: bad args (need C | 256, groups <= 64)");
    GnSeg sg{};
    sg.nlev = n_levels; sg.B = B;
    int rows = 0, chunks = 0;
    for (int l = 0; l < n_levels; ++l) {
        sg.HW[l] = HW[l]; sg.row0[l] = rows; sg.chunk0[l] = chunks; sg.nchunk[l] = ceil_div(HW[l], GN_ROWS);
        rows += B * HW[l]; chunks += B * sg.nchunk[l];
    }
    if (C == groups * 4 && 256 % groups == 0 && GN_ROWS * groups / 256 >= 1 && GN_ROWS * groups % 256 == 0 && ld % 4 == 0 && coff % 4 == 0 &&
        ((uintptr_t)x & 15) == 0) {
        const int rpt = GN_ROWS * groups / 256;
        if (x_bf16) {
            ORE_CHECK_ARG(rpt == 8, "ore_groupnorm_affine_levels_bf16_fwd: built for GroupNorm(32, 128)");
            hipLaunchKernelGGL((k_gn_chunk_stats4<8, ore_bf16_t>), dim3(chunks), dim3(256), 0, st, (const ore_bf16_t*)xv, ld, coff, sg, groups, workspace);
        } else
        if (rpt == 8) hipLaunchKernelGGL(k_gn_chunk_stats4<8>, dim3(chunks), dim3(256), 0, st, x, ld, coff, sg, groups, workspace);
        else if (rpt == 4) hipLaunchKernelGGL(k_gn_chunk_stats4<4>, dim3(chunks), dim3(256), 0, st, x, ld, coff, sg, groups, workspace);
        else hipLaunchKernelGGL(k_gn_chunk_stats, dim3(chunks), dim3(256), 0, st, x, ld, coff, sg, C, groups, workspace);
    } else {
        ORE_CHECK_ARG(!x_bf16, "ore_groupnorm_affine_levels_bf16_fwd: built for GroupNorm(32, 128)");
        hipLaunchKernelGGL(k_gn_chunk_stats, dim3(chunks), dim3(256), 0, st, x, ld, coff, sg, C, groups, workspace);
    }
    *out_sg = sg;
    return ore_launch_status("k_gn_chunk_stats");
}

static int gn_affine_levels(const void* xv, int32_t ld, int32_t coff, int32_t B, int32_t n_levels,
                                               const int32_t* HW, int32_t C, int32_t groups, float eps, const float* gamma,
                                               const float* beta, float* mul, float* add, float* workspace, void* stream, int x_bf16) {
    ORE_CHECK_ARG(gamma && beta && mul && add, "ore_groupnorm_affine_levels_fwd: null pointer");
    hipStream_t st = (hipStream_t)stream;
    GnSeg sg{};
    int rc = gn_stats_levels(xv, ld, coff, B, n_levels, HW, C, groups, workspace, st, x_bf16, &sg);
    if (rc) return rc;
    hipLaunchKernelGGL(k_gn_combine, dim3(n_levels * B), dim3(256), 0, st, workspace, sg, C, groups, eps, gamma, beta, mul, add);
    return ore_launch_status("k_gn_combine");
}

extern "C" int ore_groupnorm_affine_levels_fwd(const float* x, int32_t ld, int32_t coff, int32_t B, int32_t n_levels,
                                               const int32_t* HW, int32_t C, int32_t groups, float eps, const float* gamma,
                                               const float* beta, float* mul, float* add, float* workspace, void* stream) {
    return gn_affine_levels(x, ld, coff, B, n_levels, HW, C, groups, eps, gamma, beta, mul, add, workspace, stream, 0);
}

extern "C" int ore_groupnorm_affine_levels_bf16_fwd(const uint16_t* x, int32_t ld, int32_t coff, int32_t B, int32_t n_levels,
                                                    const int32_t* HW, int32_t C, int32_t groups, float eps, const float* gamma,
                                                    const float* beta, float* mul, float* add, float* workspace, void* stream) {
    return gn_affine_levels(x, ld, coff, B, n_levels, HW, C, groups, eps, gamma, beta, mul, add, workspace, stream, 1);
}

static int head_pred_gn(const void* tower, int32_t ld, int32_t B, int32_t n_levels, const int32_t* H, const int32_t* W, int32_t groups, float eps,
                        const float* gamma, const float* beta, const float* w_packed16, const float* scale, const float* shift,
                        int32_t ep_stride, float* out, int32_t out_ld, float* workspace, void* stream, int bf16) {
    ORE_CHECK_ARG(H && W && gamma && beta && n_levels >= 1 && n_levels <= 4, "ore_head_pred_gn_fwd: bad args");
    int32_t HW[4];
    for (int l = 0; l < n_levels; ++l) HW[l] = H[l] * W[l];
    HeadGn gn{};
    int rc = gn_stats_levels(tower, ld, 0, B, n_levels, HW, 128, groups, workspace, (hipStream_t)stream, bf16, &gn.sg);
    if (rc) return rc;
    gn.stats = workspace; gn.gamma = gamma; gn.beta = beta; gn.eps = eps; gn.G = groups;
    return head_pred_launch(tower, ld, B, n_levels, H, W, nullptr, nullptr, w_packed16, scale, shift, ep_stride, out, out_ld, stream, bf16, &gn);
}

extern "C" int ore_head_pred_gn_fwd(const float* tower, int32_t ld, int32_t B, int32_t n_levels, const int32_t* H, const int32_t* W,
                                    int32_t groups, float eps, const float* gamma, const float* beta, const float* w_packed16,
                                    const float* scale, const float* shift, int32_t ep_stride, float* out, int32_t out_ld, float* workspace,
                                    void* stream) {
    return head_pred_gn(tower, ld, B, n_levels, H, W, groups, eps, gamma, beta, w_packed16, scale, shift, ep_stride, out, out_ld, workspace, stream, 0);
}

extern "C" int ore_head_pred_gn_bf16_fwd(const uint16_t* tower, int32_t ld, int32_t B, int32_t n_levels, const int32_t* H, const int32_t* W,
                                         int32_t groups, float eps, const float* gamma, const float* beta, const float* w_packed16,
                                         const float* scale, const float* shift, int32_t ep_stride, float* out, int32_t out_ld,
                                         float* workspace, void* stream) {
    return head_pred_gn(tower, ld, B, n_levels, H, W, groups, eps, gamma, beta, w_packed16, scale, shift, ep_stride, out, out_ld, workspace, stream, 1);
}

extern "C" int ore_groupnorm_affine_fwd(const float* x, int32_t ld, int32_t coff, int32_t B, int32_t HW, int32_t C,
                                        int32_t groups, float eps, const float* gamma, const float* beta, float* mul,
                                        float* add, float* workspace, void* stream) {
    ORE_CHECK_ARG(x && gamma && beta && mul && add && workspace && groups > 0 && groups <= 64 && C % groups == 0 && C <= 256 &&
                      256 % C == 0, "ore_groupnorm_affine_fwd: bad args (need C | 256, groups <= 64)");
    const int32_t hw1[1] = {HW};
    return ore_groupnorm_affine_levels_fwd(x, ld, coff, B, 1, hw1, C, groups, eps, gamma, beta, mul, add, workspace, stream);
}

int oremisc::correlation_classes(const float* q, int32_t q_ld, int32_t q_coff, int32_t n_levels, const int32_t* H, const int32_t* W,
                                 int32_t C, int32_t K, const float* k11s, const float* k13s, const float* k31s, float* out, int32_t out_ld,
                                 void* stream) {
    ORE_CHECK_ARG(q && k11s && k13s && k31s && out && H && W && n_levels >= 1 && n_levels <= 4 && K >= 1 && K <= 16,
                  "correlation_classes: bad args");
    ORE_CHECK_ARG(C % 4 == 0 && q_ld % 4 == 0 && q_coff % 4 == 0 && out_ld % 4 == 0 && out_ld >= 2 * C, "correlation_classes: alignment");
    CorrClsP p{};
    p.q = q; p.q_ld = q_ld; p.q_coff = q_coff; p.C4 = C / 4; p.nlev = n_levels; p.K = K;
    int rows = 0;
    for (int l = 0; l < n_levels; ++l) { p.lv[l] = {rows, H[l], W[l]}; p.out_row0[l] = K * rows; rows += H[l] * W[l]; }
    p.rows = rows;
    p.k11 = k11s; p.k13 = k13s; p.k31 = k31s; p.out = out; p.out_ld = out_ld;
    hipLaunchKernelGGL(k_correlation_classes, dim3(ceil_div(p.rows * p.C4, 256)), dim3(256), 0, (hipStream_t)stream, p);
    return ore_launch_status("k_correlation_classes");
}

int oremisc::copy_cols(const float* src, int32_t src_ld, int32_t src_coff, int32_t rows, int32_t C, float* dst, int32_t dst_ld, void* stream) {
    ORE_CHECK_ARG(src && dst && rows >= 0 && C % 4 == 0 && src_ld % 4 == 0 && src_coff % 4 == 0 && dst_ld % 4 == 0, "copy_cols: bad args");
    if (rows == 0) return ORE_OK;
    hipLaunchKernelGGL(k_copy_cols, dim3(ceil_div(rows * (C / 4), 256)), dim3(256), 0, (hipStream_t)stream, src, src_ld, src_coff, rows, C / 4,
                       dst, dst_ld);
    return ore_launch_status("k_copy_cols");
}
```

### faster-orefsdet_amd/csrc/ore_util.cpp

```cpp
#include <stdarg.h>
#include <stdio.h>
#include "ore_hip.h"

static thread_local char g_err[512] = "";

void ore_set_error(const char* fmt, ...) {
    va_list ap;
    va_start(ap, fmt);
    vsnprintf(g_err, sizeof(g_err), fmt, ap);
    va_end(ap);
}

extern "C" const char* ore_last_error(void) { return g_err; }

#include <atomic>
static std::atomic<double> g_flops{0.0};
static std::atomic<long long> g_flop_calls{0};
void ore_flop_count_add(double flops) {
    double cur = g_flops.load(std::memory_order_relaxed);
    while (!g_flops.compare_exchange_weak(cur, cur + flops, std::memory_order_relaxed)) {}
    g_flop_calls.fetch_add(1, std::memory_order_relaxed);
}
static thread_local int g_last_wino = 0;
void ore_note_wino(int v) { g_last_wino = v; }
int ore_last_wino(void) { return g_last_wino; }
static thread_local int g_last_launch = ORE_LAUNCH_NONE, g_last_split = 1;
void ore_note_launch(int code, int split) { g_last_launch = code; g_last_split = split; }
extern "C" int32_t ore_conv_last_launch(int32_t* split) {
    if (split) *split = g_last_split;
    return g_last_launch;
}
extern "C" int ore_flop_counter_read(double* flops, int64_t* calls, int32_t reset) {
    if (flops) *flops = g_flops.load(std::memory_order_relaxed);
    if (calls) *calls = (int64_t)g_flop_calls.load(std::memory_order_relaxed);
    if (reset) { g_flops.store(0.0, std::memory_order_relaxed); g_flop_calls.store(0, std::memory_order_relaxed); }
    return ORE_OK;
}
extern "C" double ore_dwpw_flops(int64_t rows, int32_t C) { return 2.0 * (double)rows * (double)C * (9.0 + (double)C); }
extern "C" int32_t ore_det_record_rows(void) { return ORE_DET_RECORD_ROWS; }
extern "C" int ore_version(void) { return 601; }
```

### faster-orefsdet_amd/orehip/__init__.py

```python
from __future__ import annotations

import contextlib
import ctypes as C
import os
import re
import subprocess
from typing import Dict, List, Optional, Sequence, Tuple

import numpy as np
import torch

_PKG = os.path.dirname(os.path.dirname(os.path.abspath(__file__)))
LIB_PATH = os.path.join(_PKG, "lib", "libore_hip.so")
CSRC = os.path.join(_PKG, "csrc")
HEADER = os.path.join(os.path.dirname(_PKG), "include", "ore_hip.h")
ESE_PARTS = 512


class OreError(RuntimeError):
    pass


def build(verbose: bool = False) -> str:
    out = subprocess.run(["make", "-C", CSRC, "-j8"], capture_output=True, text=True)
# ... 488 lines not shown
    try:
        for c in codes:
            c = tuple(c) + (0,) * (5 - len(c))
            _chk(lib().ore_conv_set_plan_override(*c), "ore_conv_set_plan_override")
        yield
    finally:
        lib().ore_conv_reset_plan_overrides()


def _detect_spec(L: int, pre_topk: int):
    cap = L * pre_topk
    capa = (cap + 3) // 4 * 4
    spec = (("pre_boxes", torch.float32, 4 * capa, (cap, 4)), ("pre_scores", torch.float32, capa, (cap,)),
            ("pre_loc", torch.int64, capa, (cap,)), ("pre_level", torch.int32, capa, (cap,)), ("keep_idx", torch.int64, capa, (cap,)),
            ("counts", torch.int32, 4, (4,)), ("out_boxes", torch.float32, 4 * capa, (cap, 4)), ("out_scores", torch.float32, capa, (cap,)))
    return spec, sum(n * (8 if dt == torch.int64 else 4) for _, dt, n, _ in spec)


def _detect_desc(heads: Sequence[torch.Tensor], strides, score_thresh, pre_topk, nms_thresh, post_topk, d: "DetectDesc",
                 raw: Optional[torch.Tensor] = None, ws: Optional[torch.Tensor] = None):
    L = len(heads)
    dev = heads[0].device
    cap = L * pre_topk
    spec, raw_bytes = _detect_spec(L, pre_topk)
    if raw is None:
        raw = torch.zeros(raw_bytes, dtype=torch.uint8, device=dev)
    o, off = {}, 0
    for name, dt, n, shape in spec:
        nb = n * (8 if dt == torch.int64 else 4)
        o[name] = raw[off:off + nb].view(dt)[: shape[0] * (4 if len(shape) == 2 else 1)].view(shape)
        off += nb
    wsb = lib().ore_detect_workspace_bytes(L, pre_topk)
    if ws is None:
        ws = torch.empty(wsb, dtype=torch.uint8, device=dev)
    d.n_levels, d.head_ld = L, heads[0].shape[-1]
    for l, h in enumerate(heads):
        _f32(h)
        assert h.dim() == 3 and h.shape[-1] == d.head_ld
        d.head[l], d.H[l], d.W[l], d.stride[l] = _ptr(h), h.shape[0], h.shape[1], strides[l]
    d.score_thresh, d.pre_topk, d.nms_thresh, d.post_topk = score_thresh, pre_topk, nms_thresh, post_topk
    for k in ("pre_boxes", "pre_scores", "pre_loc", "pre_level", "keep_idx", "counts", "out_boxes", "out_scores"):
        setattr(d, k, _ptr(o[k]))
    d.workspace, d.workspace_bytes = _ptr(ws), wsb
    o["_ws"] = ws
    return o


def detect(heads: Sequence[torch.Tensor], strides: Sequence[int], score_thresh: float, pre_topk: int, nms_thresh: float,
           post_topk: int) -> Dict[str, torch.Tensor]:
    d = DetectDesc()
    o = _detect_desc(heads, strides, score_thresh, pre_topk, nms_thresh, post_topk, d)
    _chk(lib().ore_detect_fwd(C.byref(d), _stream()), "ore_detect_fwd")
    return o


def detect_batch(heads_per_image: Sequence[Sequence[torch.Tensor]], strides: Sequence[int], score_thresh: float, pre_topk: int,
                 nms_thresh: float, post_topk: int) -> List[Dict[str, torch.Tensor]]:
    B = len(heads_per_image)
    ds = (DetectDesc * B)()
    L = len(heads_per_image[0])
    _, raw_bytes = _detect_spec(L, pre_topk)
    raw_bytes = (raw_bytes + 255) // 256 * 256
    wsb = (int(lib().ore_detect_workspace_bytes(L, pre_topk)) + 255) // 256 * 256
    dev = heads_per_image[0][0].device
    raw = torch.zeros(B, raw_bytes, dtype=torch.uint8, device=dev)
    ws = torch.empty(B, wsb, dtype=torch.uint8, device=dev)
    outs = [_detect_desc(heads_per_image[b], strides, score_thresh, pre_topk, nms_thresh, post_topk, ds[b], raw[b], ws[b]) for b in range(B)]
    _chk(lib().ore_detect_batch_fwd(ds, B, _stream()), "ore_detect_batch_fwd")
    return outs


class CocoEvalDesc(C.Structure):
    _fields_ = [("n_images", C.c_int32), ("n_cats", C.c_int32),
                ("det_boxes", C.c_void_p), ("det_scores", C.c_void_p), ("det_image", C.c_void_p), ("det_cat", C.c_void_p), ("n_dets", C.c_int32),
                ("gt_boxes", C.c_void_p), ("gt_area", C.c_void_p), ("gt_crowd", C.c_void_p), ("gt_id", C.c_void_p), ("gt_off", C.c_void_p),
                ("n_gts", C.c_int32),
                ("iou_thrs_host", C.c_void_p), ("n_iou_thrs", C.c_int32), ("rec_thrs_host", C.c_void_p), ("n_rec_thrs", C.c_int32),
                ("area_rngs_host", C.c_void_p), ("n_areas", C.c_int32), ("max_dets_host", C.c_void_p), ("n_max_dets", C.c_int32),
                ("precision", C.c_void_p), ("recall", C.c_void_p), ("scores", C.c_void_p),
                ("workspace", C.c_void_p), ("workspace_bytes", C.c_size_t)]


class CocoEvalImages(C.Structure):
    _fields_ = [("n_units", C.c_void_p), ("unit_pair", C.c_void_p), ("det_index", C.c_void_p), ("dt_matches", C.c_void_p),
                ("dt_ignore", C.c_void_p), ("gt_npig", C.c_void_p), ("capacity", C.c_int64)]


def coco_eval(det_boxes: torch.Tensor, det_scores: torch.Tensor, det_image: torch.Tensor, det_cat: torch.Tensor, gt: Dict[str, torch.Tensor],
              n_images: int, n_cats: int, iou_thrs, rec_thrs, area_rngs, max_dets, per_image: bool = False,
              workspace: Optional[torch.Tensor] = None) -> Dict[str, torch.Tensor]:
    dev = det_boxes.device
    N, G = int(det_scores.numel()), int(gt["area"].numel())
    iou = np.ascontiguousarray(iou_thrs, dtype=np.float64)
    rec = np.ascontiguousarray(rec_thrs, dtype=np.float64)
    area = np.ascontiguousarray(area_rngs, dtype=np.float64).reshape(-1, 2)
    mdet = np.ascontiguousarray(max_dets, dtype=np.int32)
    T, R, A, M = len(iou), len(rec), len(area), len(mdet)
    wsb = lib().ore_coco_eval_workspace_bytes(n_cats, n_images, N, G, T, A, int(mdet[-1]))
    if wsb == 0:
        raise OreError(f"coco_eval: bad sizes (cats {n_cats}, images {n_images}, dets {N}, gts {G}, T {T}, A {A})")
    if workspace is None or workspace.numel() < wsb:
        workspace = torch.empty(wsb, dtype=torch.uint8, device=dev)
    out = {"precision": torch.empty(T, R, n_cats, A, M, dtype=torch.float64, device=dev),
           "recall": torch.empty(T, n_cats, A, M, dtype=torch.float64, device=dev),
           "scores": torch.empty(T, R, n_cats, A, M, dtype=torch.float64, device=dev)}
    det_boxes, det_scores = det_boxes.float().contiguous(), det_scores.float().contiguous()
# ... 2194 lines not shown
    def detect_classes_begin(self, img: torch.Tensor, out_h: int, out_w: int) -> torch.Tensor:
        assert img.is_contiguous() and img.dim() == 3
        _, H, W = img.shape
        R = self.__dict__.get("_rec_rows") or self.__dict__.setdefault("_rec_rows", int(lib().ore_det_record_rows()))
        rec = torch.empty(R * 7, dtype=torch.float32, device=self.device)
        _chk(lib().ore_engine_detect_classes_begin(self._h, img.data_ptr(), int(img.dtype == torch.uint8), H, W, int(out_h), int(out_w),
                                                   rec.data_ptr(), _stream()), "ore_engine_detect_classes_begin")
        return rec

    def detect_classes(self, img: torch.Tensor, out_h: int, out_w: int) -> Tuple[torch.Tensor, torch.Tensor, torch.Tensor]:
        return self.detect_end(self.detect_classes_begin(img, out_h, out_w))

    def eval_classes_forward(self, img: torch.Tensor, use_graph: bool = True) -> None:
        assert img.is_cuda and img.is_contiguous() and img.dim() == 3
        _, H, W = img.shape
        _chk(lib().ore_engine_eval_classes_fwd(self._h, img.data_ptr(), int(img.dtype == torch.uint8), H, W, int(use_graph), _stream()),
             "ore_engine_eval_classes_fwd")

    def detect_end(self, rec: torch.Tensor) -> Tuple[torch.Tensor, torch.Tensor, torch.Tensor]:
        n = C.c_int32(0)
        _chk(lib().ore_engine_detect_end(self._h, _stream(), C.byref(n)), "ore_engine_detect_end")
        k, R = n.value, self._rec_rows
        return rec.as_strided((k, 4), (4, 1)), rec.as_strided((k,), (1,), R * 4), rec.view(torch.int64).as_strided((k,), (1,), R * 5 // 2)

    def detect(self, img: torch.Tensor, out_h: int, out_w: int) -> Tuple[torch.Tensor, torch.Tensor, torch.Tensor]:
        return self.detect_end(self.detect_begin(img, out_h, out_w))

    def eval_forward_batch(self, imgs: torch.Tensor, use_graph: bool = True) -> None:
        assert imgs.is_cuda and imgs.is_contiguous() and imgs.dim() == 4
        B, _, H, W = imgs.shape
        _chk(lib().ore_engine_eval_batch_fwd(self._h, imgs.data_ptr(), int(imgs.dtype == torch.uint8), B, H, W, int(use_graph), _stream()),
             "ore_engine_eval_batch_fwd")

    def last_flops(self) -> float:
        return float(lib().ore_engine_last_flops(self._h))

    def set_profiling(self, enable: bool) -> None:
        _chk(lib().ore_engine_set_profiling(self._h, int(enable)), "ore_engine_set_profiling")

    def read_profile(self) -> Tuple[float, float, int]:
        ms, fl, n = C.c_double(), C.c_double(), C.c_int32()
        _chk(lib().ore_engine_read_profile(self._h, C.byref(ms), C.byref(fl), C.byref(n)), "ore_engine_read_profile")
        return ms.value, fl.value, n.value

    def profile_executed_flops(self) -> float:
        return float(lib().ore_engine_profile_executed_flops(self._h))

    def buffer(self, name: str, bhw: Optional[Tuple[int, int, int]] = None) -> torch.Tensor:
        p = C.c_void_p()
        dims = (C.c_int64 * 4)()
        _chk(lib().ore_engine_buffer(self._h, name.encode(), C.byref(p), dims), f"ore_engine_buffer({name})")
        rows, ch, ld, coff = (int(x) for x in dims)
        dt = {"pre_loc": torch.int64, "keep_idx": torch.int64, "pre_level": torch.int32, "counts": torch.int32, "det_src": torch.int64,
              "det_count": torch.int32, "roi_ok": torch.int32,
              "final_classes": torch.int64}.get(name.split("#")[0], torch.float32)
        if lib().ore_engine_buffer_is_bf16(self._h, name.encode()):
            dt = torch.bfloat16
        flat = _from_ptr(p.value, rows * ld, dt, self.device)
        t = flat.view(rows, ld)[:, coff:coff + ch]
        if bhw is not None:
            B, H, W = bhw
            assert B * H * W == rows, (bhw, rows)
            t = t.reshape(B, H, W, ch) if coff == 0 and ch == ld else flat.view(B, H, W, ld)[..., coff:coff + ch]
            return t.permute(0, 3, 1, 2)
        return t

    def buffer_dims(self, name: str) -> Tuple[int, int, int, int, int]:
        p, dims = C.c_void_p(), (C.c_int64 * 4)()
        _chk(lib().ore_engine_buffer(self._h, name.encode(), C.byref(p), dims), f"ore_engine_buffer({name})")
        return (p.value,) + tuple(int(x) for x in dims)

    def last_geometry(self) -> dict:
        g = (C.c_int32 * 16)()
        _chk(lib().ore_engine_last_geometry(self._h, g), "ore_engine_last_geometry")
        return {"B": g[0], "H": g[1], "W": g[2], "levels": [(g[3 + 3 * l], g[4 + 3 * l], g[5 + 3 * l]) for l in range(3)],
                "serial": int(g[12]) | (int(g[13]) << 31)}

    def heat_source(self, kind: str, slot: int = 0) -> "HeatSource":
        what = heat_kind(kind)
        geo = self.last_geometry()
        if geo["serial"] == 0:
            raise OreError("heat_source: this engine has not run a pass yet")
        if isinstance(slot, bool) or not isinstance(slot, (int, np.integer)) or not 0 <= int(slot) < geo["B"]:
            raise OreError(f"heat_source: slot {slot!r}: the last pass has {geo['B']} image(s) / class slot(s)")
        src = HeatSource.__new__(HeatSource)
        src.hw, src.strides, src.ptrs, src.ld, src.coff, src._keep = [], [], [], [], [], []
        chs, bf16 = set(), set()
        for name in what["buffers"]:
            h, w, s = geo["levels"][int(name[-1]) - 3]
            ptr, rows, ch, ld, coff = self.buffer_dims(name)
            if rows != geo["B"] * h * w:
                raise OreError(f"heat_source: buffer {name} has {rows} rows, the geometry says {geo['B']} x {h} x {w}")
            src.hw.append((h, w)); src.strides.append(s); src.ptrs.append(ptr); src.ld.append(ld); src.coff.append(coff)
            chs.add(ch)
            bf16.add(bool(lib().ore_engine_buffer_is_bf16(self._h, name.encode())))
        assert len(chs) == 1 and len(bf16) == 1, (chs, bf16)
        src.in_hw, src.batch, src.slot, src.ch, src.kind = (geo["H"], geo["W"]), geo["B"], int(slot), chs.pop(), kind
        src.device, src.is_bf16 = self.device, bf16.pop()
        src.engine, src.serial = self, geo["serial"]
        _heatmap_geometry(src.hw, src.strides, src.in_hw)
        src._set_what(what["channel"], what["transform"], what["norm"])
        return src

    def proposals(self, b: int = 0) -> Tuple[torch.Tensor, torch.Tensor, torch.Tensor]:
        n = int(self.buffer(f"counts#{b}")[1, 0].item())
        return self.buffer(f"out_boxes#{b}")[:n], self.buffer(f"out_scores#{b}")[:n, 0], self.buffer(f"keep_idx#{b}")[:n, 0]

# ... 12 lines not shown
```

### include/ore_hip.h

```cpp
#ifndef ORE_HIP_H_
#define ORE_HIP_H_
#include <stddef.h>
#include <stdint.h>
#ifdef __cplusplus
extern "C" {
#endif

#define ORE_OK 0
#define ORE_EINVAL (-22)
#define ORE_ENOMEM (-12)
#define ORE_EHIP (-5)
#define ORE_ENOENT (-2)

const char* ore_last_error(void);
int ore_version(void);
int ore_flop_counter_read(double* flops, int64_t* calls, int32_t reset);


typedef struct ore_conv_desc {
    const float* in;   int32_t in_ld, in_coff;
    int32_t B, H, W, Cin;
    const float* w;
    int32_t Cout, kh, kw, stride, pad;
    const float* scale;
// ... 69 lines not shown

int ore_stem1_fwd(const void* img, int32_t img_is_u8, int32_t B, int32_t H, int32_t W, int32_t Hp, int32_t Wp,
                  const float* mean3_host, const float* std3_host, const float* w_oihw, const float* scale,
                  const float* shift, int32_t Cout, float* out, int32_t out_ld, int32_t out_coff, void* stream);

int ore_maxpool3x3s2_fwd(const float* in, int32_t in_ld, int32_t in_coff, int32_t B, int32_t H, int32_t W,
                         int32_t C, const float* in_mul, float* out, int32_t out_ld, int32_t out_coff,
                         void* stream);

#define ORE_ESE_PARTS 512
int ore_ese_gate_fwd(const float* x, int32_t ld, int32_t coff, int32_t B, int32_t HW, int32_t C,
                     const float* fc_w, const float* fc_b, float* gate, float* workspace, void* stream);

int ore_ese_gate_from_colsum_fwd(const float* part, int32_t P, int32_t B, int32_t HW, int32_t C,
                                 const float* fc_w, const float* fc_b, float* gate, float* mean_ws, void* stream);
int ore_ese_gate_scaled_weight_fwd(const float* part, int32_t P, int32_t HW, int32_t C, const float* fc_w, const float* fc_b,
                                   float* gate, float* mean_ws, const float* w_packed, int32_t w_rows, float* w_scaled, void* stream);

int ore_scale_channels_fwd(const float* x, int32_t ld, int32_t coff, int32_t B, int32_t HW, int32_t C,
                           const float* gate, float* y, int32_t y_ld, int32_t y_coff, void* stream);

int ore_correlation_fwd(const float* q, int32_t q_ld, int32_t q_coff, int32_t B, int32_t H, int32_t W, int32_t C,
                        const float* k11, const float* k13, const float* k31,
                        float* out, int32_t out_ld, int32_t out_coff, void* stream);

int ore_correlation_levels_fwd(const float* q, int32_t q_ld, int32_t q_coff, int32_t B, int32_t n_levels,
                               const int32_t* H, const int32_t* W, int32_t C, const float* k11, const float* k13,
                               const float* k31, float* out, int32_t out_ld, int32_t out_coff, void* stream);

int ore_support_kernels_fwd(const float* proto_chw, int32_t C, int32_t s, float* k11, float* k13, float* k31,
                            void* stream);

int ore_groupnorm_affine_fwd(const float* x, int32_t ld, int32_t coff, int32_t B, int32_t HW, int32_t C,
                             int32_t groups, float eps, const float* gamma, const float* beta,
                             float* mul, float* add, float* workspace, void* stream);

int ore_groupnorm_affine_levels_fwd(const float* x, int32_t ld, int32_t coff, int32_t B, int32_t n_levels,
                                    const int32_t* HW, int32_t C, int32_t groups, float eps, const float* gamma,
                                    const float* beta, float* mul, float* add, float* workspace, void* stream);

typedef struct ore_detect_desc {
    int32_t n_levels;
    const float* head[8]; int32_t head_ld;
    int32_t H[8], W[8], stride[8];
    float score_thresh; int32_t pre_topk; float nms_thresh; int32_t post_topk;
    float* pre_boxes; float* pre_scores; int64_t* pre_loc; int32_t* pre_level;
    int64_t* keep_idx; int32_t* counts;
    float* out_boxes; float* out_scores;
    void* workspace; size_t workspace_bytes;
} ore_detect_desc;
size_t ore_detect_workspace_bytes(int32_t n_levels, int32_t pre_topk);
int ore_detect_fwd(const ore_detect_desc* d, void* stream);
int ore_detect_batch_fwd(const ore_detect_desc* d, int32_t n_images, void* stream);

size_t ore_nms_workspace_bytes(int32_t n);
int ore_nms_fwd(const float* boxes, const float* scores, int32_t n, float thr, int64_t* keep_idx,
                int32_t* count, void* workspace, size_t workspace_bytes, void* stream);

int ore_nms_device_n_fwd(const float* boxes, const float* scores, const int32_t* n_dev, int32_t cap, float thr,
                         int64_t* keep_idx, int32_t* count, void* workspace, size_t workspace_bytes, void* stream);

int ore_roi_align_fwd(const float* const* feat, const int32_t* ld, const int32_t* coff, const int32_t* H, const int32_t* W,
                      const float* scales_host, int32_t n_levels, int32_t min_level, int32_t C, int32_t pooled,
                      const float* boxes, const int32_t* n_dev, int32_t n_host, int32_t cap, float* out, void* stream);
int ore_roi_align_batched_fwd(const float* const* feat, const int32_t* ld, const int32_t* coff, const int32_t* H, const int32_t* W,
                              const float* scales_host, int32_t n_levels, int32_t min_level, int32_t C, int32_t pooled,
                              const float* boxes, const int32_t* box_image, int32_t n, float* out, void* stream);
int ore_roi_align_bwd(float* const* dfeat, const int32_t* ld, const int32_t* coff, const int32_t* H, const int32_t* W,
                      const float* scales_host, int32_t n_levels, int32_t min_level, int32_t C, int32_t pooled,
                      const float* boxes, const int32_t* box_image, int32_t n, const float* dout, void* stream);
int ore_roi_align_bwd_det(float* const* dfeat, const int32_t* ld, const int32_t* coff, const int32_t* H, const int32_t* W,
                          const float* scales_host, int32_t n_levels, int32_t min_level, int32_t C, int32_t pooled,
                          const float* boxes, const int32_t* box_image, int32_t n, const float* dout, int64_t* const* acc,
                          int32_t n_images, void* stream);

int ore_roi_align_bwd_tiled(float* const* dfeat, const int32_t* ld, const int32_t* coff, const int32_t* H, const int32_t* W,
                            const float* scales_host, int32_t n_levels, int32_t min_level, int32_t C, int32_t pooled,
                            const float* boxes, const int32_t* box_image, int32_t n, const float* dout, int32_t n_images,
                            int32_t accumulate, void* stream);
size_t ore_roi_predict_workspace_bytes(int32_t cap);
int ore_roi_predict_fwd(const float* h, int32_t C, const float* cls_w, const float* cls_b, const float* box_w,
                        const float* box_b, const float* boxes, const int32_t* n_dev, int32_t n_host, int32_t cap,
                        const float* reg_weights4_host, float img_h, float img_w, float score_thresh, float nms_thresh,
                        int32_t topk, float* det_boxes, float* det_scores, int64_t* det_src, int32_t* det_count,
                        void* workspace, size_t workspace_bytes, void* stream);
int ore_roi_predict_post_fwd(const float* h, int32_t C, const float* cls_w, const float* cls_b, const float* box_w,
                             const float* box_b, const float* boxes, const int32_t* n_dev, int32_t n_host, int32_t cap,
                             const float* reg_weights4_host, float img_h, float img_w, float score_thresh, float nms_thresh,
                             int32_t topk, float* det_boxes, float* det_scores, int64_t* det_src, int32_t* det_count,
                             const float* post_dev, float* fin_boxes, float* fin_scores, int32_t* fin_count,
                             int32_t* host_count, void* workspace, size_t workspace_bytes, void* stream);
int ore_roi_predict_parts_fwd(const float* h, int32_t C, const float* cls_w, const float* cls_b, const float* box_w,
                              const float* box_b, const float* boxes, const int32_t* n_dev, int32_t n_host, int32_t cap,
                              const float* reg_weights4_host, float img_h, float img_w, float score_thresh, float nms_thresh,
                              int32_t topk, float* det_boxes, float* det_scores, int64_t* det_src, int32_t* det_count,
                              const float* post_dev, float* fin_boxes, float* fin_scores, int32_t* fin_count,
                              int32_t* host_count, void* workspace, size_t workspace_bytes, void* stream,
                              int32_t h_parts, const float* h_bias);

int ore_roi_cascade_refine_fwd(const float* h, int32_t C, int32_t h_parts, const float* h_bias, const float* cls_w,
                               const float* cls_b, const float* box_w, const float* box_b, const float* boxes,
                               const int32_t* n_dev, int32_t n_host, int32_t cap, const float* reg_weights4_host, float img_h,
                               float img_w, float* next_boxes, float* score_sum, uint8_t* dead, int32_t accumulate, void* stream);
int ore_roi_predict_cascade_fwd(const float* h, int32_t C, const float* cls_w, const float* cls_b, const float* box_w,
                                const float* box_b, const float* boxes, const int32_t* n_dev, int32_t n_host, int32_t cap,
                                const float* reg_weights4_host, float img_h, float img_w, float score_thresh, float nms_thresh,
// ... 131 lines not shown
} ore_model_cfg;

int ore_engine_create(const ore_model_cfg* cfg, int32_t device, ore_engine** out);
void ore_engine_destroy(ore_engine* e);
int ore_engine_set_tensor(ore_engine* e, const char* name, const float* data_host, const int64_t* shape, int32_t ndim);
int ore_engine_set_support(ore_engine* e, int32_t level, const float* proto_chw_host, int32_t C, int32_t s);
int ore_engine_finalize(ore_engine* e);
int ore_engine_set_depthwise(ore_engine* e, int32_t on);
int ore_engine_set_blocks(ore_engine* e, const int32_t blocks[4]);
int ore_engine_set_roi_head(ore_engine* e, const float* W_host, const float* b_host, int32_t fc_dim, int32_t pooled,
                            const float* cls_w_host, const float* cls_b_host, const float* box_w_host, const float* box_b_host,
                            const float* reg_weights4_host, float score_thresh, float nms_thresh, int32_t topk);
#define ORE_MAX_CASCADE 4
int ore_engine_set_roi_cascade(ore_engine* e, int32_t n_stages, const float* const* W_host, const float* const* b_host,
                               int32_t fc_dim, int32_t pooled, const float* const* cls_w_host, const float* const* cls_b_host,
                               const float* const* box_w_host, const float* const* box_b_host, const float* reg_weights4_host,
                               float score_thresh, float nms_thresh, int32_t topk);

int ore_engine_backbone_fwd(ore_engine* e, const void* img, int32_t img_is_u8, int32_t B, int32_t H, int32_t W,
                            void* stream);
int ore_engine_eval_fwd(ore_engine* e, const void* img, int32_t img_is_u8, int32_t H, int32_t W, int32_t use_graph,
                        void* stream);
#define ORE_DET_RECORD_ROWS 320
#define ORE_DET_RECORD_BYTES (ORE_DET_RECORD_ROWS * 28)
int32_t ore_det_record_rows(void);
int32_t ore_engine_buffer_is_bf16(ore_engine* e, const char* name);
int ore_stem1_bf16_fwd(const void* img, int32_t img_is_u8, int32_t B, int32_t H, int32_t W, int32_t Hp, int32_t Wp, const float* mean3,
                       const float* std3, const float* w_oihw, const float* scale, const float* shift, int32_t Cout, uint16_t* out,
                       int32_t out_ld, int32_t out_coff, void* stream);
int ore_ese_gate_bf16_fwd(const uint16_t* x, int32_t ld, int32_t coff, int32_t B, int32_t HW, int32_t C, const float* fc_w,
                          const float* fc_b, float* gate, float* workspace, void* stream);
int ore_maxpool3x3s2_bf16_fwd(const uint16_t* in, int32_t in_ld, int32_t in_coff, int32_t B, int32_t H, int32_t W, int32_t C,
                              const float* in_mul, uint16_t* out, int32_t out_ld, int32_t out_coff, void* stream);
int ore_correlation_levels_bf16_fwd(const uint16_t* q, int32_t q_ld, int32_t q_coff, int32_t B, int32_t n_levels, const int32_t* H,
                                    const int32_t* W, int32_t C, const float* k11, const float* k13, const float* k31, uint16_t* out,
                                    int32_t out_ld, int32_t out_coff, void* stream);
int ore_groupnorm_affine_levels_bf16_fwd(const uint16_t* x, int32_t ld, int32_t coff, int32_t B, int32_t n_levels, const int32_t* HW,
                                         int32_t C, int32_t groups, float eps, const float* gamma, const float* beta, float* mul,
                                         float* add, float* workspace, void* stream);
int ore_groupnorm_apply_bf16_fwd(const uint16_t* x, int32_t ld, int32_t coff, int32_t images, int64_t rows_per_image, int32_t C,
                                 const float* mul_c, const float* add_c, int32_t relu, uint16_t* y, void* stream);
int ore_head_pred_fwd(const float* tower, int32_t ld, int32_t B, int32_t n_levels, const int32_t* H, const int32_t* W, const float* gn_mul,
                      const float* gn_add, const float* w_packed16, const float* scale, const float* shift, int32_t ep_stride, float* out,
                      int32_t out_ld, void* stream);
int ore_head_pred_bf16_fwd(const uint16_t* tower, int32_t ld, int32_t B, int32_t n_levels, const int32_t* H, const int32_t* W,
                           const float* gn_mul, const float* gn_add, const float* w_packed16, const float* scale, const float* shift,
                           int32_t ep_stride, float* out, int32_t out_ld, void* stream);
int ore_head_pred_gn_fwd(const float* tower, int32_t ld, int32_t B, int32_t n_levels, const int32_t* H, const int32_t* W, int32_t groups,
                         float eps, const float* gamma, const float* beta, const float* w_packed16, const float* scale, const float* shift,
                         int32_t ep_stride, float* out, int32_t out_ld, float* workspace, void* stream);
int ore_head_pred_gn_bf16_fwd(const uint16_t* tower, int32_t ld, int32_t B, int32_t n_levels, const int32_t* H, const int32_t* W,
                              int32_t groups, float eps, const float* gamma, const float* beta, const float* w_packed16, const float* scale,
                              const float* shift, int32_t ep_stride, float* out, int32_t out_ld, float* workspace, void* stream);
int ore_groupnorm_apply_levels_bf16_fwd(const uint16_t* x, int32_t ld, int32_t coff, int32_t B, int32_t n_levels, const int32_t* HW, int32_t C,
                                        const float* mul_c, const float* add_c, int32_t relu, uint16_t* y, void* stream);
int ore_ese_gate_scaled_weight_bf16_fwd(const float* part, int32_t P, int32_t HW, int32_t C, const float* fc_w, const float* fc_b,
                                        float* gate, float* mean_ws, const float* w_packed_f32, int32_t w_rows, uint16_t* w_scaled_bf16,
                                        void* stream);
int ore_ese_gate_pool_fwd(const float* part, int32_t P, int32_t HW, int32_t C, const float* fc_w, const float* fc_b, float* gate,
                          const float* w_packed, int32_t w_rows, float* w_scaled, const float* x, int32_t x_ld, int32_t x_coff,
                          int32_t H, int32_t W, float* out, int32_t out_ld, int32_t out_coff, void* stream);
int ore_ese_gate_pool_bf16_fwd(const float* part, int32_t P, int32_t HW, int32_t C, const float* fc_w, const float* fc_b, float* gate,
                               const float* w_packed_f32, int32_t w_rows, uint16_t* w_scaled_bf16, const uint16_t* x, int32_t x_ld,
                               int32_t x_coff, int32_t H, int32_t W, uint16_t* out, int32_t out_ld, int32_t out_coff, void* stream);
int ore_ese_gate_residual_fwd(const float* part, int32_t P, int32_t HW, int32_t C, const float* fc_w, const float* fc_b, float* gate,
                              const float* y, int32_t y_ld, int32_t y_coff, const float* x, int32_t x_ld, int32_t x_coff, float* out,
                              int32_t out_ld, int32_t out_coff, void* stream);
int ore_scale_residual_fwd(const float* y, int32_t y_ld, int32_t y_coff, const float* gate_bc, const float* x, int32_t x_ld, int32_t x_coff,
                           int32_t B, int32_t rows_per_image, int32_t C, float* out, int32_t out_ld, int32_t out_coff, void* stream);
int ore_roi_align_bf16_fwd(const uint16_t* const* feat, const int32_t* ld, const int32_t* coff, const int32_t* H, const int32_t* W,
                           const float* scales_host, int32_t n_levels, int32_t min_level, int32_t C, int32_t pooled, const float* boxes,
                           const int32_t* n_dev, int32_t n_host, int32_t cap, float* out, void* stream);
int ore_engine_detect_fwd(ore_engine* e, const void* img, int32_t img_is_u8, int32_t H, int32_t W, int32_t out_h, int32_t out_w,
                          void* out_record, void* stream, int32_t* n_det);
int ore_engine_detect_begin(ore_engine* e, const void* img, int32_t img_is_u8, int32_t H, int32_t W, int32_t out_h, int32_t out_w,
                            void* out_record, void* stream);
int ore_engine_detect_end(ore_engine* e, void* stream, int32_t* n_det);
int ore_engine_eval_batch_fwd(ore_engine* e, const void* img, int32_t img_is_u8, int32_t B, int32_t H, int32_t W, int32_t use_graph,
                              void* stream);
#define ORE_MAX_CLASSES 16
int ore_engine_set_classes(ore_engine* e, int32_t n, const int64_t* class_ids_host);
int ore_engine_set_support_slot(ore_engine* e, int32_t slot, int32_t level, const float* proto_chw_host, int32_t C, int32_t s);
int ore_engine_set_roi_support_slot(ore_engine* e, int32_t slot, const float* W_host, const float* b_host);
int ore_engine_set_roi_support_slot_stage(ore_engine* e, int32_t slot, int32_t stage, const float* W_host, const float* b_host);
int ore_engine_detect_classes_begin(ore_engine* e, const void* img, int32_t img_is_u8, int32_t H, int32_t W, int32_t out_h, int32_t out_w,
                                    void* out_record, void* stream);
int ore_engine_eval_classes_fwd(ore_engine* e, const void* img, int32_t img_is_u8, int32_t H, int32_t W, int32_t use_graph, void* stream);
int ore_engine_buffer(ore_engine* e, const char* name, void** dev_ptr, int64_t dims[4]);
double ore_engine_last_flops(ore_engine* e);
int ore_engine_set_profiling(ore_engine* e, int32_t enable);
int ore_engine_read_profile(ore_engine* e, double* conv_ms, double* conv_flops, int32_t* n_launches);
double ore_engine_profile_executed_flops(ore_engine* e);
int ore_event_pair_overhead_us(void* stream, int32_t reps, double* median_us);

int32_t ore_rccl_load(const char* path);
int32_t ore_rccl_unique_id(void* id128);
int32_t ore_rccl_comm_create(const void* id128, int32_t world, int32_t rank, void** comm);
int32_t ore_rccl_comm_destroy(void* comm);
int32_t ore_allreduce_grads(void* comm, float* grads, size_t count, void* stream);

typedef struct ore_coco_eval_desc {
    int32_t n_images, n_cats;
    const float* det_boxes; const float* det_scores; const int32_t* det_image; const int32_t* det_cat; int32_t n_dets;
    const double* gt_boxes; const double* gt_area; const int32_t* gt_crowd; const int64_t* gt_id; const int32_t* gt_off; int32_t n_gts;
    const double* iou_thrs_host; int32_t n_iou_thrs;
    const double* rec_thrs_host; int32_t n_rec_thrs;
// ... 147 lines not shown
```

Baseline: 1694.

## Fuse objectness sigmoid and first radix histogram pass into head prediction kernel

After: 1710 (median of 6 runs). About the same (+0.9%).

```diff
diff --git a/faster-orefsdet_amd/csrc/ore_common.h b/faster-orefsdet_amd/csrc/ore_common.h
--- a/faster-orefsdet_amd/csrc/ore_common.h
+++ b/faster-orefsdet_amd/csrc/ore_common.h
@@ -71,6 +71,7 @@
 }
 
 __device__ __forceinline__ float ore_expf(float x) {
+#pragma clang fp contract(off)
     if (x > 88.0f) x = 88.0f;
     if (x < -87.0f) x = -87.0f;
     const float n = rintf(x * 1.44269504088896341f);
@@ -87,7 +88,11 @@
     return e * __uint_as_float((unsigned)(ni + 127) << 23);
 }
 
-__device__ __forceinline__ float ore_sigmoid(float x) { return 1.0f / (1.0f + ore_expf(-x)); }
+__device__ __forceinline__ float ore_sigmoid(float x) {
+#pragma clang fp contract(off)
+    return 1.0f / (1.0f + ore_expf(-x));
+}
+__device__ __forceinline__ unsigned ore_select_digit(float s, int pass) { return (__float_as_uint(s) >> (20 - 10 * pass)) & 1023u; }
 
 namespace oreroi {
 int roi_predict_post(const float* h, int32_t C, int32_t h_parts, const float* h_bias, const float* cls_w, const float* cls_b,
diff --git a/faster-orefsdet_amd/csrc/ore_detect.hip b/faster-orefsdet_amd/csrc/ore_detect.hip
--- a/faster-orefsdet_amd/csrc/ore_detect.hip
+++ b/faster-orefsdet_amd/csrc/ore_detect.hip
@@ -23,6 +23,7 @@
     unsigned long long* mask; int mask_words;
     long long* keep_idx; int* counts; float* out_boxes; float* out_scores;
     int cap;
+    const float* score[8]; const int* hist0[8];
 };
 
 constexpr int SEL_T = 1024;
@@ -49,9 +50,40 @@
     return base + inc - v;
 }
 
+__device__ __forceinline__ int radix_pick(const int* h1024, int lane, int remaining, bool strict, int* sh_i) {
+    int h[16], t = 0;
+    const int4* hv = reinterpret_cast<const int4*>(h1024 + 16 * lane);
+#pragma unroll
+    for (int j = 0; j < 4; ++j) { const int4 q = hv[j]; h[4 * j] = q.x; h[4 * j + 1] = q.y; h[4 * j + 2] = q.z; h[4 * j + 3] = q.w; }
+#pragma unroll
+    for (int j = 0; j < 16; ++j) t += h[j];
+    int suf = t;
+#pragma unroll
+    for (int d = 1; d < 64; d <<= 1) {
+        const int o = __shfl_down(suf, d);
+        if (lane + d < 64) suf += o;
+    }
+    const int above = suf - t;
+    const int total = __shfl(suf, 0);
+    if ((!strict || total > remaining) && suf >= remaining && above < remaining) {
+        int acc = above, dsel = 0, rem = remaining;
+        bool found = false;
+#pragma unroll
+        for (int j = 15; j >= 0; --j) {
+            if (!found) {
+                if (acc + h[j] >= remaining) { dsel = j; rem = remaining - acc; found = true; }
+                else acc += h[j];
+            }
+        }
+        sh_i[0] = 16 * lane + dsel; sh_i[1] = rem;
+    }
+    return total;
+}
+
+template <bool PRE>
 __device__ __forceinline__ void level_select_body(const DetP& p) {
     extern __shared__ __attribute__((aligned(16))) float sv[];
-    __shared__ int hist[1024];
+    __shared__ __attribute__((aligned(16))) int hist[1024];
     __shared__ int wsum[SEL_T / 64];
     __shared__ int sh_i[4];
     const int l = blockIdx.x;
@@ -61,15 +93,37 @@
     const bool tr = l == 0 && tid == 0;
     if (tr) DET_TR(0);
 
-    int cnt = 0;
-    for (int i = tid; i < HW; i += SEL_T) {
-        const float s = ore_sigmoid(hd[(size_t)i * p.head_ld + 4]);
-        sv[i] = s;
-        cnt += s > p.score_thresh ? 1 : 0;
-    }
-    if (tr) DET_TR(1);
     int nc;
-    block_excl_scan(cnt, wsum, &nc);
+    if (PRE) {
+        if (tid < 64) {
+            const int tot = radix_pick(p.hist0[l], tid, p.pre_topk, true, sh_i);
+            if (tid == 0) sh_i[2] = tot;
+        } else {
+            const float* pl = p.score[l];
+            const int t = tid - 64, nt = SEL_T - 64;
+            const int lead = min((int)((4u - (unsigned)(((uintptr_t)pl >> 2) & 3u)) & 3u), HW);
+            const int nv = (HW - lead) >> 2;
+            if (t < lead) sv[t] = pl[t];
+            for (int v = t; v < nv; v += nt) {
+                const f32x4 q = *reinterpret_cast<const f32x4*>(pl + lead + 4 * v);
+                float* d = sv + lead + 4 * v;
+                d[0] = q.x; d[1] = q.y; d[2] = q.z; d[3] = q.w;
+            }
+            for (int i = lead + 4 * nv + t; i < HW; i += nt) sv[i] = pl[i];
+        }
+        if (tr) DET_TR(1);
+        __syncthreads();
+        nc = sh_i[2];
+    } else {
+        int cnt = 0;
+        for (int i = tid; i < HW; i += SEL_T) {
+            const float s = ore_sigmoid(hd[(size_t)i * p.head_ld + 4]);
+            sv[i] = s;
+            cnt += s > p.score_thresh ? 1 : 0;
+        }
+        if (tr) DET_TR(1);
+        block_excl_scan(cnt, wsum, &nc);
+    }
     if (tr) DET_TR(2);
     const int k = nc < p.pre_topk ? nc : p.pre_topk;
 
@@ -80,7 +134,10 @@
         take_all = false;
         unsigned prefix = 0, pmask = 0;
         int remaining = k;
-        for (int pass = 0; pass < 3; ++pass) {
+        if (PRE) {
+            prefix = (unsigned)sh_i[0] << 20; pmask = 1023u << 20; remaining = sh_i[1];
+        }
+        for (int pass = PRE ? 1 : 0; pass < 3; ++pass) {
             const int shift = 20 - 10 * pass;
             for (int i = tid; i < 1024; i += SEL_T) hist[i] = 0;
             __syncthreads();
@@ -90,30 +147,7 @@
                 if (s > p.score_thresh && (key & pmask) == prefix) atomicAdd(&hist[(key >> shift) & 1023], 1);
             }
             __syncthreads();
-            if (tid < 64) {
-                int h[16], t = 0;
-#pragma unroll
-                for (int j = 0; j < 16; ++j) { h[j] = hist[16 * tid + j]; t += h[j]; }
-                int suf = t;
-#pragma unroll
-                for (int d = 1; d < 64; d <<= 1) {
-                    const int o = __shfl_down(suf, d);
-                    if (tid + d < 64) suf += o;
-                }
-                const int above = suf - t;
-                if (suf >= remaining && above < remaining) {
-                    int acc = above, dsel = 0, rem = remaining;
-                    bool found = false;
-#pragma unroll
-                    for (int j = 15; j >= 0; --j) {
-                        if (!found) {
-                            if (acc + h[j] >= remaining) { dsel = j; rem = remaining - acc; found = true; }
-                            else acc += h[j];
-                        }
-                    }
-                    sh_i[0] = 16 * tid + dsel; sh_i[1] = rem;
-                }
-            }
+            if (tid < 64) radix_pick(hist, tid, remaining, false, sh_i);
             __syncthreads();
             prefix |= (unsigned)sh_i[0] << shift;
             pmask |= 1023u << shift;
@@ -170,7 +204,12 @@
     if (tr) DET_TR(8);
 }
 
-__global__ __launch_bounds__(SEL_T) void k_level_select(DetP p) { level_select_body(p); }
+__global__ __launch_bounds__(SEL_T) void k_level_select(DetP p) { level_select_body<false>(p); }
+__global__ __launch_bounds__(SEL_T) void k_level_select_pre(DetP p) { level_select_body<true>(p); }
+__global__ __launch_bounds__(256) void k_detect_sigmoid(const float* __restrict__ x, float* __restrict__ y, long long n) {
+    const long long i = (long long)blockIdx.x * 256 + threadIdx.x;
+    if (i < n) y[i] = ore_sigmoid(x[i]);
+}
 
 constexpr int DET_BATCH = 16;
 struct DetImg { const float* head[4]; char* ws; float* pre_boxes; float* pre_scores; long long* pre_loc; int* pre_level;
@@ -193,7 +232,7 @@
     p.keep_idx = m.keep_idx; p.counts = m.counts; p.out_boxes = m.out_boxes; p.out_scores = m.out_scores;
     return p;
 }
-__global__ __launch_bounds__(SEL_T) void k_level_select_b(DetBatch b) { const DetP p = det_of(b, blockIdx.y); level_select_body(p); }
+__global__ __launch_bounds__(SEL_T) void k_level_select_b(DetBatch b) { const DetP p = det_of(b, blockIdx.y); level_select_body<false>(p); }
 
 __device__ __forceinline__ void rank_scatter_body(const DetP& p) {
     extern __shared__ float sc[];
@@ -760,14 +799,30 @@
     return ORE_OK;
 }
 
-static int detect_prepare(const ore_detect_desc* d, hipStream_t st, ScanArgs& sa, DetLayout& lay, int& cap) {
+static int detect_prepare(const ore_detect_desc* d, hipStream_t st, ScanArgs& sa, DetLayout& lay, int& cap, const float* score = nullptr,
+                          const int32_t* hist0 = nullptr, int B = 1, int b = 0) {
     DetP p{};
     size_t sv_bytes = 0;
     int rc = detect_fill(d, p, lay, cap, sv_bytes);
     if (rc) return rc;
-    if (sv_bytes > 48 * 1024)
-        ORE_HIP(hipFuncSetAttribute((const void*)k_level_select, hipFuncAttributeMaxDynamicSharedMemorySize, (int)sv_bytes));
-    hipLaunchKernelGGL(k_level_select, dim3(d->n_levels), dim3(SEL_T), sv_bytes, st, p);
+    if (score) {
+        ORE_CHECK_ARG(hist0 && ((uintptr_t)hist0 & 15) == 0 && ((uintptr_t)score & 3) == 0 && B >= 1 && b >= 0 && b < B,
+                      "ore_detect_prepaid_fwd: null or misaligned plane / histogram, or image %d of %d", b, B);
+        size_t row0 = 0;
+        for (int l = 0; l < d->n_levels; ++l) {
+            const size_t HW = (size_t)d->H[l] * d->W[l];
+            p.score[l] = score + row0 + (size_t)b * HW;
+            p.hist0[l] = hist0 + ((size_t)l * B + b) * 1024;
+            row0 += (size_t)B * HW;
+        }
+        if (sv_bytes > 48 * 1024)
+            ORE_HIP(hipFuncSetAttribute((const void*)k_level_select_pre, hipFuncAttributeMaxDynamicSharedMemorySize, (int)sv_bytes));
+        hipLaunchKernelGGL(k_level_select_pre, dim3(d->n_levels), dim3(SEL_T), sv_bytes, st, p);
+    } else {
+        if (sv_bytes > 48 * 1024)
+            ORE_HIP(hipFuncSetAttribute((const void*)k_level_select, hipFuncAttributeMaxDynamicSharedMemorySize, (int)sv_bytes));
+        hipLaunchKernelGGL(k_level_select, dim3(d->n_levels), dim3(SEL_T), sv_bytes, st, p);
+    }
     if ((rc = ore_launch_status("k_level_select"))) return rc;
     const size_t sc_bytes = (size_t)cap * 4;
     if (sc_bytes > 64 * 1024)
@@ -823,15 +878,30 @@
 
 }
 
-extern "C" int ore_detect_fwd(const ore_detect_desc* d, void* stream) {
+static int detect_one(const ore_detect_desc* d, void* stream, const float* score, const int32_t* hist0, int B, int b) {
     ScanArgs sa{};
     DetLayout lay{};
     int cap = 0;
     hipStream_t st = (hipStream_t)stream;
-    const int rc = detect_prepare(d, st, sa, lay, cap);
+    const int rc = detect_prepare(d, st, sa, lay, cap, score, hist0, B, b);
     if (rc) return rc;
     return launch_nms_scan(lay.words, st, sa.s_boxes, sa.s_scores, sa.s_order, sa.n_ptr, sa.mask, d->nms_thresh, d->post_topk, sa.keep_idx,
                            sa.out_boxes, sa.out_scores, sa.n_keep_out, nms_use_col(cap) ? nms_col_ld(cap) : 0);
+}
+
+extern "C" int ore_detect_fwd(const ore_detect_desc* d, void* stream) { return detect_one(d, stream, nullptr, nullptr, 1, 0); }
+
+extern "C" int ore_detect_prepaid_fwd(const ore_detect_desc* d, const float* score, const int32_t* hist0, int32_t B, int32_t b, void* stream) {
+    ORE_CHECK_ARG(score && hist0, "ore_detect_prepaid_fwd: null score plane or histogram");
+    return detect_one(d, stream, score, hist0, B, b);
+}
+
+extern "C" int ore_detect_sigmoid_fwd(const float* x, float* y, int64_t n, void* stream) {
+    ORE_CHECK_ARG((x && y) || n == 0, "ore_detect_sigmoid_fwd: null pointer");
+    ORE_CHECK_ARG(n >= 0 && n < (1ll << 31) * 256, "ore_detect_sigmoid_fwd: n %lld", (long long)n);
+    if (n == 0) return ORE_OK;
+    hipLaunchKernelGGL(k_detect_sigmoid, dim3((unsigned)((n + 255) / 256)), dim3(256), 0, (hipStream_t)stream, x, y, (long long)n);
+    return ore_launch_status("k_detect_sigmoid");
 }
 
 extern "C" int ore_detect_batch_fwd(const ore_detect_desc* d, int32_t n_images, void* stream) {
diff --git a/faster-orefsdet_amd/csrc/ore_engine.hip b/faster-orefsdet_amd/csrc/ore_engine.hip
--- a/faster-orefsdet_amd/csrc/ore_engine.hip
+++ b/faster-orefsdet_amd/csrc/ore_engine.hip
@@ -76,6 +76,9 @@
     float* pre_boxes = nullptr; float* pre_scores = nullptr; int64_t* pre_loc = nullptr; int32_t* pre_level = nullptr;
     int64_t* keep_idx = nullptr; int32_t* counts = nullptr; float* out_boxes = nullptr; float* out_scores = nullptr;
     void* det_ws = nullptr; size_t det_ws_bytes = 0;
+    bool select_prepaid = true;
+    float* sel_score = nullptr; int32_t* sel_hist0 = nullptr;
+    bool prepaid() const { return select_prepaid && cfg.fpn_ch == 128 && head_pred_valu; }
     bool roi_set = false;
     int roi_cap = ORE_DET_RECORD_ROWS, roi_fc = 0, roi_pooled = 8, roi_topk = 100;
     float roi_score_thresh = 0.f, roi_nms_thresh = 0.9f, roi_reg_w[4] = {10.f, 10.f, 5.f, 5.f};
@@ -474,7 +477,7 @@
     return r.rc;
 }
 
-int run_heads(ore_engine* e, const Geo& g, hipStream_t st, double* flops, bool correlate = true) {
+int run_heads(ore_engine* e, const Geo& g, hipStream_t st, double* flops, bool correlate = true, bool prepay = false) {
     const ore_model_cfg& c = e->cfg;
     const int F = c.fpn_ch;
     Run r{e, st};
@@ -496,10 +499,14 @@
     r.conv_levels(e->tower, e->pos.p, F, 0, g.B, H, W, e->tow.p, F, 0);
     if (r.rc) return r.rc;
     if (F == 128 && e->head_pred_valu) {
-        r.rc = sb ? ore_head_pred_gn_bf16_fwd(reinterpret_cast<const uint16_t*>(e->tow.p), F, g.B, 3, H, W, 32, 1e-5f, e->gn_gamma, e->gn_beta,
-                                              e->pred.w, e->pred.scale, e->pred.shift, 16, e->head.p, 8, e->gn_ws, st)
-                  : ore_head_pred_gn_fwd(e->tow.p, F, g.B, 3, H, W, 32, 1e-5f, e->gn_gamma, e->gn_beta, e->pred.w, e->pred.scale,
-                                         e->pred.shift, 16, e->head.p, 8, e->gn_ws, st);
+        if (prepay && e->prepaid())
+            r.rc = ore_head_pred_gn_select_fwd(e->tow.p, sb ? 1 : 0, F, g.B, 3, H, W, 32, 1e-5f, e->gn_gamma, e->gn_beta, e->pred.w, e->pred.scale,
+                                               e->pred.shift, 16, e->head.p, 8, e->gn_ws, e->sel_score, e->sel_hist0, c.score_thresh, st);
+        else
+            r.rc = sb ? ore_head_pred_gn_bf16_fwd(reinterpret_cast<const uint16_t*>(e->tow.p), F, g.B, 3, H, W, 32, 1e-5f, e->gn_gamma, e->gn_beta,
+                                                  e->pred.w, e->pred.scale, e->pred.shift, 16, e->head.p, 8, e->gn_ws, st)
+                      : ore_head_pred_gn_fwd(e->tow.p, F, g.B, 3, H, W, 32, 1e-5f, e->gn_gamma, e->gn_beta, e->pred.w, e->pred.scale,
+                                             e->pred.shift, 16, e->head.p, 8, e->gn_ws, st);
         r.flops += 2.0 * rows * 5.0 * F * 9.0;
         *flops = r.flops;
         return r.rc;
@@ -540,6 +547,7 @@
 int run_detect(ore_engine* e, const Geo& g, hipStream_t st, int b = 0) {
     ore_detect_desc d{};
     detect_desc(e, g, b, d);
+    if (e->prepaid()) return ore_detect_prepaid_fwd(&d, e->sel_score, e->sel_hist0, g.B, b, st);
     return ore_detect_fwd(&d, st);
 }
 
@@ -753,6 +761,7 @@
     e->cfg = *cfg; e->device = device;
     e->conv_precision = ore_conv_get_precision();
     { const char* hm = getenv("ORE_HEAD_MFMA"); e->head_pred_valu = !(hm && hm[0] == '1'); }
+    { const char* sp = getenv("ORE_SELECT_PREPAID"); e->select_prepaid = !(sp && sp[0] == '0'); }
     *out = e;
     return ORE_OK;
 }
@@ -982,6 +991,7 @@
         (rc = alloc_buf(e, &e->tow, rows_all, F)) || (rc = alloc_buf(e, &e->head, rows_all, 8, false))) return rc;
     if (e->sb() && (rc = alloc_buf(e, &e->tn, rows_all, F))) return rc;
     ORE_HIP(hipMemset(e->head.p, 0, rows_all * 8 * sizeof(float)));
+    if ((rc = e->dalloc(&e->sel_score, rows_all)) || (rc = e->dalloc(&e->sel_hist0, (size_t)3 * B * 1024))) return rc;
     if ((rc = e->dalloc(&e->gn_mul, 3 * B * F)) || (rc = e->dalloc(&e->gn_add, 3 * B * F))) return rc;
     if ((rc = e->dalloc(&e->k11, (size_t)3 * F)) || (rc = e->dalloc(&e->k13, (size_t)3 * F * 3)) || (rc = e->dalloc(&e->k31, (size_t)3 * F * 3))) return rc;
     e->ws_floats = ore_conv_workspace_floats();
@@ -1139,7 +1149,7 @@
         double f1 = 0, f2 = 0;
         int r = run_backbone(e, e->img_in, is_u8, g, s, &f1);
         double f3 = 0;
-        if (!r) r = run_heads(e, g, s, &f2);
+        if (!r) r = run_heads(e, g, s, &f2, true, true);
         for (int b = 0; b < B && !r; ++b) {
             double fb = 0;
             r = run_detect(e, g, s, b);
@@ -1380,6 +1390,10 @@
         if (n == "pos" + k) return set(e->at(e->pos.p, r0 * F), rows, F, F, 0);
         if (n == "tower" + k) return set(e->at(e->tow.p, r0 * F), rows, F, F, 0);
         if (n == "head" + k) return set(e->head.p + r0 * 8, rows, 5, 8, 0);
+        if (e->prepaid()) {
+            if (n == "sel_score" + k) return set(e->sel_score + r0, rows, 1, 1, 0);
+            if (n == "sel_hist" + k) return set(e->sel_hist0 + (size_t)l * g.B * 1024, g.B, 1024, 1024, 0);
+        }
     }
     size_t ib = 0;
     std::string base = n;
diff --git a/faster-orefsdet_amd/csrc/ore_misc.hip b/faster-orefsdet_amd/csrc/ore_misc.hip
--- a/faster-orefsdet_amd/csrc/ore_misc.hip
+++ b/faster-orefsdet_amd/csrc/ore_misc.hip
@@ -451,9 +451,12 @@
 
 template <int RPT, typename TS = float>
 __global__ __launch_bounds__(256) void k_gn_chunk_stats4(const TS* __restrict__ x, int ld, int coff, GnSeg sg, int G,
-                                                         float* __restrict__ stats ) {
+                                                         float* __restrict__ stats ,
+                                                         int* __restrict__ zero = nullptr, int zero_n = 0) {
     __shared__ float red[256];
     __shared__ float gmean[64];
+    if (zero)
+        for (int i = blockIdx.x * 256 + threadIdx.x; i < zero_n; i += gridDim.x * 256) zero[i] = 0;
     int seg, HW, row0, chunk;
     gn_locate_chunk(sg, blockIdx.x, seg, HW, row0, chunk);
     const int g = threadIdx.x % G, rr = threadIdx.x / G, rpar = 256 / G;
@@ -566,6 +569,9 @@
     const float* scale; const float* shift; int ep_stride;
     float* out; int out_ld;
     const float* stats; GnSeg sg; const float* gamma; const float* beta; float eps; int G;
+    float* score;
+    int* hist0;
+    float score_thresh;
 };
 
 template <typename TS>
@@ -586,6 +592,7 @@
     const TS* tow = reinterpret_cast<const TS*>(p.tow);
     __shared__ __attribute__((aligned(16))) float s_mul[C], s_add[C];
     __shared__ GnCombineSm S;
+    __shared__ int s_bin[TP * TP];
     constexpr int NX = (HP * HP * Q + 255) / 256;
     constexpr int NWV = (NO * 9 * Q + 255) / 256;
     f32x4 xv[NX], wv[NWV];
@@ -665,10 +672,31 @@
         for (int k = 0; k < Q; k += 4) { s0 += pp[k]; s1 += pp[k + 1]; s2 += pp[k + 2]; s3 += pp[k + 3]; }
         float v = (s0 + s1) + (s2 + s3);
         const int gy = y0 + px / TP, gx = x0 + px % TP;
+        int bin = -1;
         if (gy < H && gx < W) {
             v = v * p.scale[lvl * p.ep_stride + o] + p.shift[lvl * p.ep_stride + o];
             if (o < 4) v = fmaxf(v, 0.f);
             p.out[(size_t)(base + gy * W + gx) * p.out_ld + o] = v;
+            if (o == 4 && p.score) {
+                const float s = ore_sigmoid(v);
+                p.score[base + gy * W + gx] = s;
+                if (s > p.score_thresh) bin = (int)ore_select_digit(s, 0);
+            }
+        }
+        if (o == 4) s_bin[px] = bin;
+    }
+    if (p.score) {
+        __syncthreads();
+        if (tid < TP * TP) {
+            const int mine = s_bin[tid];
+            int n = 0, lowest = TP * TP;
+#pragma unroll
+            for (int j = TP * TP - 1; j >= 0; --j) {
+                const bool same = s_bin[j] == mine;
+                n += same ? 1 : 0;
+                lowest = same ? j : lowest;
+            }
+            if (mine >= 0 && lowest == tid) atomicAdd(&p.hist0[(lvl * p.B + b) * 1024 + mine], n);
         }
     }
 }
@@ -678,7 +706,8 @@
 struct HeadGn { const float* stats; GnSeg sg; const float* gamma; const float* beta; float eps; int G; };
 static int head_pred_launch(const void* tower, int32_t ld, int32_t B, int32_t n_levels, const int32_t* H, const int32_t* W, const float* mul,
                             const float* add, const float* w_packed16, const float* scale, const float* shift, int32_t ep_stride,
-                            float* out, int32_t out_ld, void* stream, int bf16, const HeadGn* gn = nullptr) {
+                            float* out, int32_t out_ld, void* stream, int bf16, const HeadGn* gn = nullptr, float* score = nullptr,
+                            int32_t* hist0 = nullptr, float score_thresh = 0.f) {
     ORE_CHECK_ARG(tower && H && W && (gn || (mul && add)) && w_packed16 && scale && shift && out, "ore_head_pred_fwd: null pointer");
     ORE_CHECK_ARG(B > 0 && n_levels >= 1 && n_levels <= 4 && ld >= 128 && ld % 4 == 0 && out_ld >= 5, "ore_head_pred_fwd: bad args");
     HeadP p{};
@@ -693,6 +722,7 @@
     p.tile0[n_levels] = tiles;
     p.mul = mul; p.add = add; p.w = w_packed16; p.scale = scale; p.shift = shift; p.ep_stride = ep_stride; p.out = out; p.out_ld = out_ld;
     if (gn) { p.stats = gn->stats; p.sg = gn->sg; p.gamma = gn->gamma; p.beta = gn->beta; p.eps = gn->eps; p.G = gn->G; }
+    p.score = score; p.hist0 = hist0; p.score_thresh = score_thresh;
     if (bf16) hipLaunchKernelGGL(k_head_pred<ore_bf16_t>, dim3(tiles), dim3(256), 0, (hipStream_t)stream, p);
     else hipLaunchKernelGGL(k_head_pred<float>, dim3(tiles), dim3(256), 0, (hipStream_t)stream, p);
     return ore_launch_status("k_head_pred");
@@ -947,7 +977,7 @@
 }
 
 static int gn_stats_levels(const void* xv, int32_t ld, int32_t coff, int32_t B, int32_t n_levels, const int32_t* HW, int32_t C, int32_t groups,
-                           float* workspace, hipStream_t st, int x_bf16, GnSeg* out_sg) {
+                           float* workspace, hipStream_t st, int x_bf16, GnSeg* out_sg, int* zero = nullptr, int zero_n = 0) {
     const float* x = (const float*)xv;
     ORE_CHECK_ARG(x && HW && workspace && n_levels >= 1 && n_levels <= 4 && groups > 0 && groups <= 64 && C % groups == 0 && C <= 256 &&
                       256 % C == 0, "ore_groupnorm_affine_levels_fwd: bad args (need C | 256, groups <= 64)");
@@ -961,14 +991,16 @@
     if (C == groups * 4 && 256 % groups == 0 && GN_ROWS * groups / 256 >= 1 && GN_ROWS * groups % 256 == 0 && ld % 4 == 0 && coff % 4 == 0 &&
         ((uintptr_t)x & 15) == 0) {
         const int rpt = GN_ROWS * groups / 256;
+        ORE_CHECK_ARG(!zero || rpt == 8, "ore_head_pred_gn_select_fwd: built for GroupNorm(32, 128)");
         if (x_bf16) {
             ORE_CHECK_ARG(rpt == 8, "ore_groupnorm_affine_levels_bf16_fwd: built for GroupNorm(32, 128)");
-            hipLaunchKernelGGL((k_gn_chunk_stats4<8, ore_bf16_t>), dim3(chunks), dim3(256), 0, st, (const ore_bf16_t*)xv, ld, coff, sg, groups, workspace);
+            hipLaunchKernelGGL((k_gn_chunk_stats4<8, ore_bf16_t>), dim3(chunks), dim3(256), 0, st, (const ore_bf16_t*)xv, ld, coff, sg, groups, workspace, zero, zero_n);
         } else
-        if (rpt == 8) hipLaunchKernelGGL(k_gn_chunk_stats4<8>, dim3(chunks), dim3(256), 0, st, x, ld, coff, sg, groups, workspace);
-        else if (rpt == 4) hipLaunchKernelGGL(k_gn_chunk_stats4<4>, dim3(chunks), dim3(256), 0, st, x, ld, coff, sg, groups, workspace);
+        if (rpt == 8) hipLaunchKernelGGL(k_gn_chunk_stats4<8>, dim3(chunks), dim3(256), 0, st, x, ld, coff, sg, groups, workspace, zero, zero_n);
+        else if (rpt == 4) hipLaunchKernelGGL(k_gn_chunk_stats4<4>, dim3(chunks), dim3(256), 0, st, x, ld, coff, sg, groups, workspace, (int*)nullptr, 0);
         else hipLaunchKernelGGL(k_gn_chunk_stats, dim3(chunks), dim3(256), 0, st, x, ld, coff, sg, C, groups, workspace);
     } else {
+        ORE_CHECK_ARG(!zero, "ore_head_pred_gn_select_fwd: the tower must be 16-byte aligned with ld %% 4 == 0");
         ORE_CHECK_ARG(!x_bf16, "ore_groupnorm_affine_levels_bf16_fwd: built for GroupNorm(32, 128)");
         hipLaunchKernelGGL(k_gn_chunk_stats, dim3(chunks), dim3(256), 0, st, x, ld, coff, sg, C, groups, workspace);
     }
@@ -1002,15 +1034,28 @@
 
 static int head_pred_gn(const void* tower, int32_t ld, int32_t B, int32_t n_levels, const int32_t* H, const int32_t* W, int32_t groups, float eps,
                         const float* gamma, const float* beta, const float* w_packed16, const float* scale, const float* shift,
-                        int32_t ep_stride, float* out, int32_t out_ld, float* workspace, void* stream, int bf16) {
+                        int32_t ep_stride, float* out, int32_t out_ld, float* workspace, void* stream, int bf16, float* score = nullptr,
+                        int32_t* hist0 = nullptr, float score_thresh = 0.f) {
     ORE_CHECK_ARG(H && W && gamma && beta && n_levels >= 1 && n_levels <= 4, "ore_head_pred_gn_fwd: bad args");
+    ORE_CHECK_ARG(!score == !hist0 && (!score || B > 0), "ore_head_pred_gn_select_fwd: score and hist0 come together");
     int32_t HW[4];
     for (int l = 0; l < n_levels; ++l) HW[l] = H[l] * W[l];
     HeadGn gn{};
-    int rc = gn_stats_levels(tower, ld, 0, B, n_levels, HW, 128, groups, workspace, (hipStream_t)stream, bf16, &gn.sg);
+    int rc = gn_stats_levels(tower, ld, 0, B, n_levels, HW, 128, groups, workspace, (hipStream_t)stream, bf16, &gn.sg, hist0,
+                             hist0 ? n_levels * B * 1024 : 0);
     if (rc) return rc;
     gn.stats = workspace; gn.gamma = gamma; gn.beta = beta; gn.eps = eps; gn.G = groups;
-    return head_pred_launch(tower, ld, B, n_levels, H, W, nullptr, nullptr, w_packed16, scale, shift, ep_stride, out, out_ld, stream, bf16, &gn);
+    return head_pred_launch(tower, ld, B, n_levels, H, W, nullptr, nullptr, w_packed16, scale, shift, ep_stride, out, out_ld, stream, bf16, &gn,
+                            score, hist0, score_thresh);
+}
+
+extern "C" int ore_head_pred_gn_select_fwd(const void* tower, int32_t tower_bf16, int32_t ld, int32_t B, int32_t n_levels, const int32_t* H,
+                                           const int32_t* W, int32_t groups, float eps, const float* gamma, const float* beta,
+                                           const float* w_packed16, const float* scale, const float* shift, int32_t ep_stride, float* out,
+                                           int32_t out_ld, float* workspace, float* score, int32_t* hist0, float score_thresh, void* stream) {
+    ORE_CHECK_ARG(score && hist0, "ore_head_pred_gn_select_fwd: null score plane or histogram");
+    return head_pred_gn(tower, ld, B, n_levels, H, W, groups, eps, gamma, beta, w_packed16, scale, shift, ep_stride, out, out_ld, workspace, stream,
+                        tower_bf16 ? 1 : 0, score, hist0, score_thresh);
 }
 
 extern "C" int ore_head_pred_gn_fwd(const float* tower, int32_t ld, int32_t B, int32_t n_levels, const int32_t* H, const int32_t* W,
diff --git a/faster-orefsdet_amd/csrc/ore_util.cpp b/faster-orefsdet_amd/csrc/ore_util.cpp
--- a/faster-orefsdet_amd/csrc/ore_util.cpp
+++ b/faster-orefsdet_amd/csrc/ore_util.cpp
@@ -38,4 +38,4 @@
 }
 extern "C" double ore_dwpw_flops(int64_t rows, int32_t C) { return 2.0 * (double)rows * (double)C * (9.0 + (double)C); }
 extern "C" int32_t ore_det_record_rows(void) { return ORE_DET_RECORD_ROWS; }
-extern "C" int ore_version(void) { return 601; }
+extern "C" int ore_version(void) { return 602; }
diff --git a/faster-orefsdet_amd/orehip/__init__.py b/faster-orefsdet_amd/orehip/__init__.py
--- a/faster-orefsdet_amd/orehip/__init__.py
+++ b/faster-orefsdet_amd/orehip/__init__.py
@@ -564,6 +564,42 @@
     o = _detect_desc(heads, strides, score_thresh, pre_topk, nms_thresh, post_topk, d)
     _chk(lib().ore_detect_fwd(C.byref(d), _stream()), "ore_detect_fwd")
     return o
+
+
+def detect_prepaid(heads: Sequence[torch.Tensor], score: torch.Tensor, hist0: torch.Tensor, strides: Sequence[int], score_thresh: float,
+                   pre_topk: int, nms_thresh: float, post_topk: int, B: int = 1, b: int = 0) -> Dict[str, torch.Tensor]:
+    assert score.dtype == torch.float32 and hist0.dtype == torch.int32 and score.is_contiguous() and hist0.is_contiguous()
+    assert hist0.numel() == len(heads) * B * 1024 and score.numel() >= B * sum(h.shape[0] * h.shape[1] for h in heads)
+    d = DetectDesc()
+    o = _detect_desc(heads, strides, score_thresh, pre_topk, nms_thresh, post_topk, d)
+    _chk(lib().ore_detect_prepaid_fwd(C.byref(d), _ptr(score), _ptr(hist0), B, b, _stream()), "ore_detect_prepaid_fwd")
+    return o
+
+
+def detect_sigmoid(x: torch.Tensor) -> torch.Tensor:
+    _f32(x)
+    y = torch.empty_like(x)
+    _chk(lib().ore_detect_sigmoid_fwd(_ptr(x), _ptr(y), x.numel(), _stream()), "ore_detect_sigmoid_fwd")
+    return y
+
+
+def head_pred_gn_select(tower: torch.Tensor, B: int, levels: Sequence[Tuple[int, int]], gamma: torch.Tensor, beta: torch.Tensor,
+                        w_packed16: torch.Tensor, scale: torch.Tensor, shift: torch.Tensor, score_thresh: float, out_ld: int = 8,
+                        hist0: Optional[torch.Tensor] = None) -> Tuple[torch.Tensor, torch.Tensor, torch.Tensor]:
+    rows, ld = tower.shape
+    assert rows == B * sum(h * w for h, w in levels) and tower.is_contiguous() and tower.dtype in (torch.float32, torch.bfloat16)
+    dev = tower.device
+    out = torch.zeros(rows, out_ld, device=dev)
+    score = torch.full((rows,), float("nan"), device=dev)
+    if hist0 is None:
+        hist0 = torch.full((len(levels) * B, 1024), -7, dtype=torch.int32, device=dev)
+    assert hist0.dtype == torch.int32 and hist0.numel() == len(levels) * B * 1024 and hist0.is_contiguous()
+    ws = torch.empty(sum(B * ((h * w + 63) // 64) for h, w in levels) * 32 * 2 + 64, device=dev)
+    _chk(lib().ore_head_pred_gn_select_fwd(_ptr(tower), 1 if tower.dtype == torch.bfloat16 else 0, ld, B, len(levels),
+                                           _i32s([h for h, _ in levels]), _i32s([w for _, w in levels]), 32, 1e-5, _ptr(gamma), _ptr(beta),
+                                           _ptr(w_packed16), _ptr(scale), _ptr(shift), scale.shape[1], _ptr(out), out_ld, _ptr(ws),
+                                           _ptr(score), _ptr(hist0), score_thresh, _stream()), "ore_head_pred_gn_select_fwd")
+    return out, score, hist0
 
 
 def detect_batch(heads_per_image: Sequence[Sequence[torch.Tensor]], strides: Sequence[int], score_thresh: float, pre_topk: int,
@@ -2864,7 +2900,7 @@
         _chk(lib().ore_engine_buffer(self._h, name.encode(), C.byref(p), dims), f"ore_engine_buffer({name})")
         rows, ch, ld, coff = (int(x) for x in dims)
         dt = {"pre_loc": torch.int64, "keep_idx": torch.int64, "pre_level": torch.int32, "counts": torch.int32, "det_src": torch.int64,
-              "det_count": torch.int32, "roi_ok": torch.int32,
+              "det_count": torch.int32, "roi_ok": torch.int32, "sel_hist3": torch.int32, "sel_hist4": torch.int32, "sel_hist5": torch.int32,
               "final_classes": torch.int64}.get(name.split("#")[0], torch.float32)
         if lib().ore_engine_buffer_is_bf16(self._h, name.encode()):
             dt = torch.bfloat16
diff --git a/include/ore_hip.h b/include/ore_hip.h
--- a/include/ore_hip.h
+++ b/include/ore_hip.h
@@ -145,6 +145,8 @@
 size_t ore_detect_workspace_bytes(int32_t n_levels, int32_t pre_topk);
 int ore_detect_fwd(const ore_detect_desc* d, void* stream);
 int ore_detect_batch_fwd(const ore_detect_desc* d, int32_t n_images, void* stream);
+int ore_detect_prepaid_fwd(const ore_detect_desc* d, const float* score, const int32_t* hist0, int32_t B, int32_t b, void* stream);
+int ore_detect_sigmoid_fwd(const float* x, float* y, int64_t n, void* stream);
 
 size_t ore_nms_workspace_bytes(int32_t n);
 int ore_nms_fwd(const float* boxes, const float* scores, int32_t n, float thr, int64_t* keep_idx,
@@ -382,6 +384,10 @@
 int ore_head_pred_gn_bf16_fwd(const uint16_t* tower, int32_t ld, int32_t B, int32_t n_levels, const int32_t* H, const int32_t* W,
                               int32_t groups, float eps, const float* gamma, const float* beta, const float* w_packed16, const float* scale,
                               const float* shift, int32_t ep_stride, float* out, int32_t out_ld, float* workspace, void* stream);
+int ore_head_pred_gn_select_fwd(const void* tower, int32_t tower_bf16, int32_t ld, int32_t B, int32_t n_levels, const int32_t* H,
+                                const int32_t* W, int32_t groups, float eps, const float* gamma, const float* beta, const float* w_packed16,
+                                const float* scale, const float* shift, int32_t ep_stride, float* out, int32_t out_ld, float* workspace,
+                                float* score, int32_t* hist0, float score_thresh, void* stream);
 int ore_groupnorm_apply_levels_bf16_fwd(const uint16_t* x, int32_t ld, int32_t coff, int32_t B, int32_t n_levels, const int32_t* HW, int32_t C,
                                         const float* mul_c, const float* add_c, int32_t relu, uint16_t* y, void* stream);
 int ore_ese_gate_scaled_weight_bf16_fwd(const float* part, int32_t P, int32_t HW, int32_t C, const float* fc_w, const float* fc_b,
```
